# xipengwang/AprilSAM

Hardware: AMD Instinct MI355X
Metric: Gauss-Newton iterations/sec + factorise ms on M3500 (chi2 match <=1e-6) (higher is better)
Workload: dtype f64; 1 GPU; M3500 batch april_graph_cholesky, 1 replica per GPU (3500 poses, 5454 factors, n=10500); parallelism=single GPU, fronts=680, levels=9, nnz_L=422121

## Files before the change

### aprilsam_amd/csrc/capi.cpp

```cpp
#include <cstdio>
#include <cstdlib>
#include <cstring>
#include <string>
#include <vector>

#include "../../include/aprilsam_amd.h"
#include "plan.h"
#include "errors.h"
#include "refmodel.h"
#include "solver.h"

extern "C" {

void APRILSAM_VERSION(void) {
    printf("================\n");
    printf("| APRILSAM 0.0 |   solver: aprilsam_amd (MI355X / gfx950)\n");
    printf("================\n");
    printf("\n");
}

void april_graph_cholesky_param_init(april_graph_cholesky_param_t *param) {
    asam::drop_context(param);
    asam::unbind_param(param);
    memset(param, 0, sizeof(*param));
    param->tikhanov = 0.0001;
    param->nreordering = 1;
    asam::warm_up();
}

void april_graph_cholesky_param_destory(april_graph_cholesky_param_t *param) {
    if (!param) return;
    asam::drop_context(param);
    asam::unbind_param(param);
    free(param->delta_x); free(param->B); free(param->y); free(param->ordering);
    free(param);
}

void april_graph_cholesky(april_graph_t *graph, april_graph_cholesky_param_t *param) { asam::batch_step(graph, param); }

void april_graph_cholesky_inc(april_graph_t *graph, april_graph_cholesky_param_t *param) { asam::inc_step(graph, param); }

void april_graph_cholesky_inc_solver(april_graph_t *graph, april_graph_cholesky_param_t *param, int *idxs) {
    (void)idxs;
    asam::inc_solve_only(graph, param);
}

double april_graph_chi2(april_graph_t *graph) { return asam::graph_chi2(graph); }

int aprilsam_amd_device_count(void) { return asam::api_device_count(); }
int aprilsam_amd_set_device(int device) { return asam::api_set_device(device); }
int aprilsam_amd_param_set_device(const april_graph_cholesky_param_t *param, int slot) { return asam::api_param_set_device(param, slot); }
int aprilsam_amd_param_get_device(const april_graph_cholesky_param_t *param) { return asam::api_param_get_device(param); }
int aprilsam_amd_set_option(const char *name, double value) { return asam::api_set_option(name, value); }
int aprilsam_amd_debug_guard_selftest(const april_graph_cholesky_param_t *param) { return asam::debug_guard_selftest(param); }
int aprilsam_amd_get_option(const char *name, double *value) { return asam::api_get_option(name, value); }
int aprilsam_amd_get_stats(const april_graph_cholesky_param_t *param, aprilsam_amd_stats_t *out) {
    return asam::get_stats(param, out) ? 0 : -1;
}
int aprilsam_amd_batch_resident(april_graph_t *graph, april_graph_cholesky_param_t *param, int iters, double *chi2_out, double *ms_out) {
    return asam::batch_resident(graph, param, iters, chi2_out, ms_out);
}
int aprilsam_amd_resident_begin(april_graph_t *graph, april_graph_cholesky_param_t *param) { return asam::resident_begin(graph, param); }
int aprilsam_amd_resident_steps(april_graph_t *graph, april_graph_cholesky_param_t *param, int n, int mode) { return asam::resident_steps(graph, param, n, mode); }
int aprilsam_amd_resident_sync(april_graph_t *graph, april_graph_cholesky_param_t *param) { return asam::resident_sync(graph, param); }
double aprilsam_amd_resident_chi2(april_graph_t *graph) { return asam::resident_chi2(graph); }
int aprilsam_amd_resident_end(april_graph_t *graph, april_graph_cholesky_param_t *param) { return asam::resident_end(graph, param); }
int aprilsam_amd_level_profile(const april_graph_cholesky_param_t *param, double *out6, int cap_levels) { return asam::level_profile(param, out6, cap_levels); }
int aprilsam_amd_kernel_profile(const april_graph_cholesky_param_t *param, double *ms, long long *calls, double *flops, double *bytes, const char **names) {
    return asam::kernel_profile(param, ms, calls, flops, bytes, names);
}
int aprilsam_amd_debug_stage(april_graph_t *graph, april_graph_cholesky_param_t *param, int what, double *out) { return asam::debug_stage(graph, param, what, out); }
int aprilsam_amd_debug_front_times(const april_graph_cholesky_param_t *param, long long *out, int n_fronts) { return asam::debug_front_times(param, out, n_fronts); }
int aprilsam_amd_reference_order(int n_nodes, int n_factors, const int *fa, const int *fb, int *out_order, int *out_parent) {
    asam::RefModel m;
    m.batch(n_nodes, n_factors, fa, fb);
    memcpy(out_order, m.ord.data(), sizeof(int) * (size_t)n_nodes);
    if (out_parent) memcpy(out_parent, m.parent.data(), sizeof(int) * (size_t)n_nodes);
    return 0;
}
int aprilsam_amd_shard_begin(april_graph_t *graph, april_graph_cholesky_param_t *param, int rank, int world) { return asam::shard_begin(graph, param, rank, world); }
long long aprilsam_amd_shard_info(const april_graph_cholesky_param_t *param, int what, long long *out, long long cap) { return asam::shard_info(param, what, out, cap); }
int aprilsam_amd_shard_comm_unique_id(char *out128) { return asam::shard_comm_unique_id(out128); }
int aprilsam_amd_shard_comm_init_rccl(april_graph_cholesky_param_t *param, const char *id128) { return asam::shard_comm_init_rccl(param, id128); }
int aprilsam_amd_shard_comm_init_host(april_graph_cholesky_param_t *param, const aprilsam_amd_host_comm_t *cb) { return asam::shard_comm_init_host(param, cb); }
int aprilsam_amd_shard_comm_info(const april_graph_cholesky_param_t *param, long long *out5, char *rccl_path, int cap) { return asam::shard_comm_info(param, out5, rccl_path, cap); }
int aprilsam_amd_shard_iterate(april_graph_t *graph, april_graph_cholesky_param_t *param, int n) { return asam::shard_iterate(graph, param, n); }
int aprilsam_amd_shard_gather_states(april_graph_t *graph, april_graph_cholesky_param_t *param) { return asam::shard_gather_states(graph, param); }
double aprilsam_amd_shard_chi2(april_graph_t *graph, april_graph_cholesky_param_t *param) { return asam::shard_chi2(graph, param); }
void aprilsam_amd_shard_end(april_graph_cholesky_param_t *param) { asam::shard_end(param); }

void *aprilsam_amd_refmodel_create(void) { return new asam::RefModel(); }
void aprilsam_amd_refmodel_destroy(void *m) { delete (asam::RefModel *)m; }
void aprilsam_amd_refmodel_batch(void *m, int n_nodes, int n_factors, const int *fa, const int *fb) { ((asam::RefModel *)m)->batch(n_nodes, n_factors, fa, fb); }
int aprilsam_amd_refmodel_inc_begin(void *m, int n_nodes, int n_factors, const int *fa, const int *fb) {
    asam::RefModel *M = (asam::RefModel *)m;
    M->inc_begin(n_nodes, n_factors, fa, fb);
    return M->naffected;
}
int aprilsam_amd_refmodel_solve_visit(void *m, const double *x, double dxy, double dth, int *visited) {
    asam::RefModel *M = (asam::RefModel *)m;
    for (int i = 0; i < M->N; i++) visited[i] = 0;
    M->solve_visit(x, dxy, dth, [&](int n, bool upd) { visited[n] = upd ? 2 : 1; });
    return M->start_over;
}
void aprilsam_amd_refmodel_get(void *m, int *parent, int *changed, int *relin) {
    asam::RefModel *M = (asam::RefModel *)m;
    for (int i = 0; i < M->N; i++) { if (parent) parent[i] = M->parent[i]; if (changed) changed[i] = M->changed[i]; if (relin) relin[i] = M->relin[i]; }
}
int aprilsam_amd_refmodel_check(void *m) { return ((asam::RefModel *)m)->check_tree(); }
int aprilsam_amd_last_error(char *msg, int cap) { return asam::get_last_error(msg, cap); }
void aprilsam_amd_clear_error(void) { asam::clear_last_error(); }
int aprilsam_amd_selftest(void) { return asam::selftest(); }
const char *aprilsam_amd_version(void) { return "aprilsam_amd 0.1 (gfx950, multifrontal FP64)"; }
void aprilsam_amd_free(void *p) { free(p); }

struct aprilsam_amd_plan { asam::Plan P; };

aprilsam_amd_plan_t *aprilsam_amd_plan_create(int n_nodes, int n_factors, const int *factor_nodes, const double *xy, int leaf_nodes) {
    aprilsam_amd_plan *pl = new aprilsam_amd_plan();
    try {
        asam::build_plan(pl->P, n_nodes, n_factors, factor_nodes, xy, leaf_nodes > 0 ? leaf_nodes : asam::g_opt.leaf_nodes);
    } catch (const asam::SolverError &e) {
        asam::set_last_error(e.code, e.msg);
        fprintf(stderr, "aprilsam_amd: ERROR %d: %s\n", e.code, e.msg.c_str());
        delete pl;
        return nullptr;
    } catch (const std::exception &e) {
        asam::set_last_error(asam::ERR_INTERNAL, e.what());
        fprintf(stderr, "aprilsam_amd: ERROR %d: %s\n", (int)asam::ERR_INTERNAL, e.what());
        delete pl;
        return nullptr;
    }
    return pl;
}
void aprilsam_amd_plan_destroy(aprilsam_amd_plan_t *plan) { delete plan; }

long long aprilsam_amd_shard_plan(const aprilsam_amd_plan_t *plan, int world, int what, long long *out, long long cap) {
    if (!plan || world < 1) return -1;
    std::vector<int> owner; std::vector<char> top; std::vector<long long> xfer, bcast, v;
    asam::shard_map(plan->P, world, owner, top, xfer, bcast);
    if (what == 1) v = xfer; else if (what == 2) v = bcast; else if (what == 3) v.assign(owner.begin(), owner.end());
    else if (what == 4) v = asam::shard_critical_path(plan->P, world, owner, top); else return -1;
    if (out) for (long long i = 0; i < (long long)v.size() && i < cap; i++) out[i] = v[i];
    return (long long)v.size();
}

long long aprilsam_amd_plan_query(const aprilsam_amd_plan_t *plan, const char *what, long long **out) {
    std::string k(what);
    if (k.compare(0, 3, "bd_") == 0 || k.compare(0, 3, "rd_") == 0) asam::build_gather_lists(const_cast<asam::Plan &>(plan->P));
    const asam::Plan &P = plan->P;
    std::vector<long long> v;
    auto from = [&](const auto &a) { v.assign(a.begin(), a.end()); };
    if (k == "perm") from(P.perm);
    else if (k == "pos") from(P.pos);
    else if (k == "front_first") from(P.f_first);
    else if (k == "front_nsb") from(P.f_nsb);
    else if (k == "front_nub") from(P.f_nub);
    else if (k == "front_parent") from(P.f_parent);
    else if (k == "front_level") from(P.f_level);
    else if (k == "front_rows_ptr") from(P.f_rows_ptr);
    else if (k == "front_rows") from(P.f_rows);
    else if (k == "front_rel") from(P.f_rel);
    else if (k == "front_off") from(P.f_off);
    else if (k == "ch_ptr") from(P.ch_ptr);
    else if (k == "ch_idx") from(P.ch_idx);
    else if (k == "factor_front") from(P.fac_front);
    else if (k == "factor_la") from(P.fac_la);
    else if (k == "factor_lb") from(P.fac_lb);
    else if (k == "factor_swap") from(P.fac_swap);
    else if (k == "bd_front_ptr") from(P.bd_front_ptr);
    else if (k == "bd_row") from(P.bd_row);
    else if (k == "bd_col") from(P.bd_col);
    else if (k == "bd_src_ptr") from(P.bd_src_ptr);
    else if (k == "bd_src") from(P.bd_src);
    else if (k == "rd_front_ptr") from(P.rd_front_ptr);
    else if (k == "rd_col") from(P.rd_col);
    else if (k == "rd_src_ptr") from(P.rd_src_ptr);
    else if (k == "rd_src") from(P.rd_src);
    else if (k == "lev_ptr") from(P.lev_ptr);
    else if (k == "lev_fronts") from(P.lev_fronts);
    else if (k == "stats") v = { P.nF, P.nLevels, P.max_rows, (long long)P.nnzL, (long long)P.flops, (long long)P.pool_doubles };
    else { *out = nullptr; return -1; }
    *out = (long long *)malloc(sizeof(long long) * (v.size() + 1));
    if (!v.empty()) memcpy(*out, v.data(), sizeof(long long) * v.size());
    return (long long)v.size();
}

}
```

### aprilsam_amd/csrc/kernels.hip.h

```cpp
#pragma once
#include <hip/hip_runtime.h>
#include <stdint.h>

#include <type_traits>
namespace asam {

constexpr int PROF_SLOTS = 16;
constexpr int TPB = 256;
constexpr int NB = 32;
constexpr int TILE = 64;
constexpr int ASM_CB = 4;
constexpr int OBP = 4;

struct FrontDesc {
    long long off;
    int nsb, nub, first;
    int dest_begin, dest_end;
    int ch_begin, ch_end;
    int rows_begin;
    int parent;
    int dinv0;
    int prim1, prim2;
    int pad[2];
};
static_assert(sizeof(FrontDesc) == 64, "FrontDesc must stay one cache line");
struct DestRec { int brow, bcol, src_begin, src_end; };
struct ChildRec {
    long long uoff;
    int cR;
    int cnu;
    int rel_begin;
    int pad;
};
static_assert(sizeof(ChildRec) == 24, "ChildRec layout");

struct DevPlan {
    int nF;
    const FrontDesc *fd;
    const DestRec *dest;
    const ChildRec *child;
    const int *f_rows, *f_rel;
    const int *slot_blk, *slot_rhs;
    const int *src_idx;
    const double *lambda;
    long long *prof;
    int prof_mode;
    int schur_first_nub;
    int *epoch; const int *flevel; int l0; const int *marks;
};

__host__ __device__ inline int asm_chunks(int nbc) { return (nbc + ASM_CB - 1) / ASM_CB; }
struct SyrkRange { int k_lo, k_hi, col_lo, col_hi, ntr, ntc; };
__host__ __device__ inline SyrkRange syrk_range(int R, int C, int ns, int s_lo, int s_hi, int tile = TILE, bool ahead = false) {
    SyrkRange g;
    g.k_lo = s_lo * NB;
    g.k_hi = s_hi * NB < ns ? s_hi * NB : ns;
    g.col_lo = g.k_hi;
    g.col_hi = ahead ? (g.k_hi + OBP * NB < ns ? g.k_hi + OBP * NB : ns) : C;
    if (g.k_hi <= g.k_lo || g.col_hi <= g.col_lo) { g.ntr = g.ntc = 0; return g; }
    g.ntr = ((R - 2) - g.col_lo + tile - 1) / tile;
    g.ntc = (g.col_hi - g.col_lo + tile - 1) / tile;
    return g;
}
__host__ __device__ inline int syrk_tiles(int R, int C, int ns, int s_lo, int s_hi, int tile = TILE, bool ahead = false) {
    SyrkRange g = syrk_range(R, C, ns, s_lo, s_hi, tile, ahead);
    return g.ntc * g.ntr - g.ntc * (g.ntc - 1) / 2;
}
__device__ __forceinline__ int find_seg(const int *__restrict__ pre, int n, int bid) {
    int lo = 0, hi = n;
    while (hi - lo > 1) { int m = (lo + hi) >> 1; if (pre[m] <= bid) lo = m; else hi = m; }
    return lo;
}

__device__ __forceinline__ void trapezoid_tile(int l, int ntr, int ntc, int *ti, int *tj_);
constexpr int SYRK_SB = 8;
constexpr int SYRK_MODE_XCD_SHIFT = 8;
__host__ __device__ inline void trapezoid_tile_xcd(int l, int nt, int ntr, int ntc, int *ti, int *tj) {
    const int q = nt >> 3, rem = nt & 7, x = l & 7;
    int lp = x * q + (x < rem ? x : rem) + (l >> 3);
    for (int c0 = 0;; ) {
        const int w = ntc - c0 < SYRK_SB ? ntc - c0 : SYRK_SB;
        const int cnt = w * (ntr - c0) - w * (w - 1) / 2;
        if (lp < cnt || c0 + w >= ntc) {
            const int tri = w * (w + 1) / 2;
            if (lp < tri) { int r = 0; while ((r + 1) * (r + 2) / 2 <= lp) r++; *ti = c0 + r; *tj = c0 + lp - r * (r + 1) / 2; }
            else { const int e = lp - tri; *ti = c0 + w + e / w; *tj = c0 + e % w; }
            return;
        }
        lp -= cnt; c0 += w;
    }
// ... 735 lines not shown
        }
    }
}
template <int BWT>
__device__ __forceinline__ void chain_store_diag(double *S, int ld, int k0, int wdt, const double (&Dd)[BWT]) {
    const int r = threadIdx.x & 63;
    if (r < wdt) {
#pragma unroll
        for (int c = 0; c < BWT; c++) if (c < wdt) S[(k0 + c) * ld + k0 + r] = (c <= r) ? Dd[c] : 0.0;
    }
}
template <int NT>
__device__ __forceinline__ void factor_dense_blk(double *S, int ld, int ns, int Rv, int hi, int *bad, double * , long long *pf = nullptr) {
    constexpr int NW = NT / 64;
    long long t_chain = 0, t_syrk = 0, t0 = 0;
    const int wave = __builtin_amdgcn_readfirstlane(threadIdx.x >> 6);
    auto chain_sync_store = [&](int k0, int nwc) {
        const int wdt = min(BW, ns - k0);
        if (wdt <= 8) {
            double D8[8];
            chain_block<NT, 8>(S, ld, k0, wdt, Rv, bad, D8, nwc);
            __syncthreads();
            if (wave == 0) chain_store_diag<8>(S, ld, k0, wdt, D8);
        } else {
            double D16[16];
            chain_block<NT, 16>(S, ld, k0, wdt, Rv, bad, D16, nwc);
            __syncthreads();
            if (wave == 0) chain_store_diag<16>(S, ld, k0, wdt, D16);
        }
    };
    auto chain_waves = [&](int k0) {
        const int wdt = min(BW, ns - k0), brows = 64 - (wdt <= 8 ? 8 : 16);
        const int nchunk = max(1, (Rv - (k0 + wdt) + brows - 1) / brows);
        return min(nchunk, NW / 2);
    };
    if (pf) t0 = wall_clock64();
    chain_sync_store(0, NW);
    if (pf) { const long long t1 = wall_clock64(); t_chain += t1 - t0; t0 = t1; }
    for (int k0 = 0; k0 < ns; k0 += BW) {
        const int wdt = min(BW, ns - k0), below0 = k0 + wdt;
        if (below0 < ns) {
            const int next_hi = min(below0 + BW, ns), cw = chain_waves(below0);
            if (NW >= 8) lds_syrk16<NT>(S, ld, k0, below0, below0, next_hi, Rv, 1, NW - 1);
            else lds_syrk16<NT>(S, ld, k0, below0, below0, next_hi, Rv);
            __syncthreads();
            if (pf) { const long long t1 = wall_clock64(); t_syrk += t1 - t0; t0 = t1; }
            if (wave < cw) {
                long long w0_ = 0, c0_ = 0;
                if (pf) { w0_ = wall_clock64(); c0_ = clock64(); }
                chain_sync_store(below0, cw);
                if (pf && threadIdx.x == 0) { pf[10] += clock64() - c0_; pf[15] += wall_clock64() - w0_; }
            } else {
                if (next_hi < hi) lds_syrk16<NT>(S, ld, k0, below0, next_hi, hi, Rv, cw, NW - cw);
                __syncthreads();
            }
            if (pf) { const long long t1 = wall_clock64(); t_chain += t1 - t0; t0 = t1; }
        } else {
            __syncthreads();
            if (below0 < hi) lds_syrk16<NT>(S, ld, k0, below0, below0, hi, Rv);
            __syncthreads();
            if (pf) { const long long t1 = wall_clock64(); t_syrk += t1 - t0; t0 = t1; }
        }
    }
    if (pf && threadIdx.x == 0) { pf[8] = t_chain; pf[9] = t_syrk; }
}
template <int NT>
__device__ __forceinline__ void factor_front_blk(double *S, int ld, int nsb, int nbc, int *bad, double *stage, int nbc_upd = -1, long long *pf = nullptr) {
    if (nbc_upd < 0) nbc_upd = nbc;
    factor_dense_blk<NT>(S, ld, 3 * nsb, 3 * (nbc + 1) - 2, 3 * nbc_upd, bad, stage, pf);
}

__host__ __device__ inline size_t small_front_lds(int R, int C, int nw) { return (size_t)(R | 1) * C * 8 + wl_bytes(nw); }
__host__ __device__ inline size_t panel_front_lds(int R, int ns, int nw) { return (size_t)(R | 1) * ns * 8 + wl_bytes(nw); }

template <int NT>
__device__ __forceinline__ void front_small_body(const DevPlan &P, const int t, double *__restrict__ pool, const double *__restrict__ Hc, int *bad,
                                                 long long full_lds_limit, int *flags, int wait, double *S) {
    const int *wflags = wait ? flags : nullptr;
    const int ev = flags ? flag_value(P) : 0;
    const FrontDesc D = P.fd[t];
    const int nsb = D.nsb, nbc = D.nsb + D.nub;
    const int R = 3 * (nbc + 1), C = 3 * nbc, ld = R | 1;
    double *Fg = pool + D.off;
    if ((long long)small_front_lds(R, C, NT / 64) <= full_lds_limit) {
        int2 *wl = (int2 *)(S + (size_t)ld * C);
        if (P.prof && threadIdx.x == 0) P.prof[(size_t)t * PROF_SLOTS + 0] = wall_clock64();
        assemble_front<NT, ASM_LDS>(P, D, pool, Hc, 0, nbc, true, S, ld, nullptr, 0, wl, P.prof ? P.prof + (size_t)t * PROF_SLOTS : nullptr, wflags, bad, ev);
        if (P.prof && threadIdx.x == 0) P.prof[(size_t)t * PROF_SLOTS + 1] = wall_clock64();
        factor_front_blk<NT>(S, ld, nsb, nbc, bad, (double *)wl, -1, P.prof ? P.prof + (size_t)t * PROF_SLOTS : nullptr);
        if (P.prof && threadIdx.x == 0) P.prof[(size_t)t * PROF_SLOTS + 2] = wall_clock64();
        for (int c = 3 * nsb + (threadIdx.x >> 6); c < C; c += NT / 64) {
            int r0 = 3 * (c / 3);
            for (int r = r0 + (threadIdx.x & 63); r < R; r += 64) Fg[(size_t)c * R + r] = S[(size_t)c * ld + r];
        }
        if (flags) publish_flag(flags + t, ev);
        for (int c = threadIdx.x >> 6; c < 3 * nsb; c += NT / 64) {
            int r0 = 3 * (c / 3);
            for (int r = r0 + (threadIdx.x & 63); r < R; r += 64) Fg[(size_t)c * R + r] = S[(size_t)c * ld + r];
        }
    } else {
        const int ns = 3 * nsb;
        int2 *wl = (int2 *)(S + (size_t)ld * ns);
        const bool schur_first = P.schur_first_nub > 0 && D.nub >= P.schur_first_nub;
        if (P.prof && threadIdx.x == 0) P.prof[(size_t)t * PROF_SLOTS + 0] = wall_clock64();
        if (schur_first) assemble_front<NT, ASM_SPLIT>(P, D, pool, Hc, 0, nsb, false, S, ld, Fg, R, wl, P.prof ? P.prof + (size_t)t * PROF_SLOTS : nullptr, wflags, bad, ev);
        else assemble_front<NT, ASM_SPLIT>(P, D, pool, Hc, 0, nbc, true, S, ld, Fg, R, wl, P.prof ? P.prof + (size_t)t * PROF_SLOTS : nullptr, wflags, bad, ev);
        if (P.prof && threadIdx.x == 0) P.prof[(size_t)t * PROF_SLOTS + 1] = wall_clock64();
        factor_front_blk<NT>(S, ld, nsb, nbc, bad, (double *)wl, nsb, P.prof ? P.prof + (size_t)t * PROF_SLOTS : nullptr);
        if (P.prof && threadIdx.x == 0) P.prof[(size_t)t * PROF_SLOTS + 2] = wall_clock64();
        if (schur_first) {
            lds_panel_syrk<NT, 2>(S, ld, 0, ns, ns, C, R - 2, Fg, R);
            __syncthreads();
            assemble_front<NT, ASM_GLOBAL, false>(P, D, pool, Hc, nsb, nbc, false, nullptr, 0, Fg, R, wl, nullptr, nullptr, bad);
        }
        else if (nbc > nsb) lds_panel_syrk<NT, 1>(S, ld, 0, ns, ns, C, R - 2, Fg, R);
        if (flags) publish_flag(flags + t, ev);
        for (int c = threadIdx.x >> 6; c < ns; c += NT / 64) {
            int r0 = 3 * (c / 3);
            for (int r = r0 + (threadIdx.x & 63); r < R; r += 64) Fg[(size_t)c * R + r] = S[(size_t)c * ld + r];
        }
    }
    if (P.prof) { __syncthreads(); if (threadIdx.x == 0) P.prof[(size_t)t * PROF_SLOTS + 3] = wall_clock64(); }
}
constexpr int UPD_MAXF = 4;
constexpr int UPD_MAXC = 4;
struct UpdRec {
    long long old_off;
    int mode;
    int old_nub;
    int wout;
    int mask;
    int n_own, own_f[UPD_MAXF], own_la[UPD_MAXF], own_lb[UPD_MAXF], own_slot[UPD_MAXF];
    int n_ch, ch_t[UPD_MAXC], ch_wout[UPD_MAXC], ch_rel[UPD_MAXC], ch_cnu[UPD_MAXC], ch_mask[UPD_MAXC];
    int pad[3];
};
static_assert(sizeof(UpdRec) == 192, "UpdRec layout");
struct UpdCtx {
    const UpdRec *recs;
    double *wbuf;
    int *wflags;
    const int *fa, *fb; const double *Z, *Wm, *lp, *st;
};
__host__ __device__ inline size_t update_front_lds(int R, int ns, int nact) {
    return (size_t)((size_t)ns * (R | 1) + (size_t)3 * nact * (R | 1) + 8 * ns + 3 * (ns | 1) + 16) * 8;
}
template <int NT>
__device__ __forceinline__ void front_update_body(const DevPlan &P, const int t, const UpdRec &rec, const UpdCtx &uc, double *__restrict__ pool,
                                                  int *flags, int *bad, double *S) {
    constexpr int NW = NT / 64;
    const FrontDesc D = P.fd[t];
    const int tid = threadIdx.x, wave = __builtin_amdgcn_readfirstlane(tid >> 6), lane = tid & 63;
    const int ns = 3 * D.nsb, nu = 3 * D.nub, m = ns + nu, R = m + 3, ld = R | 1;
    const int nu_o = 3 * rec.old_nub, m_o = ns + nu_o, R_o = m_o + 3;
    const double *Fo = pool + rec.old_off;
    double *Fg = pool + D.off;
    const int nact = __popc(rec.mask), wld = nu + 1, nsp = ns | 1;
    double *Ls = S;
    double *Wv = Ls + (size_t)ns * ld;
    double *K8 = Wv + (size_t)3 * nact * ld;
    double *Wa = K8 + 8 * ns;
    double *Cm = Wa + 3 * nsp;
    long long *pf = P.prof ? P.prof + (size_t)t * PROF_SLOTS : nullptr;
    if (pf && tid == 0) pf[0] = wall_clock64();
    const int ev = (flags || uc.wflags) ? flag_value(P) : 0;
    {
        const int ne = ns * R;
// ... 170 lines not shown
#pragma unroll
                    for (int u = 0; u < 4; u++) { L[u] = Li[(size_t)(j + u) * ld]; pp[3 * u] = K8[8 * (j + u)]; pp[3 * u + 1] = K8[8 * (j + u) + 1]; pp[3 * u + 2] = K8[8 * (j + u) + 2]; }
#pragma unroll
                    for (int u = 0; u < 4; u++) { r0 = fma(-L[u], pp[3 * u], r0); r1 = fma(-L[u], pp[3 * u + 1], r1); r2 = fma(-L[u], pp[3 * u + 2], r2); }
                }
                for (; j < ns; j++) { const double L = Li[(size_t)j * ld]; r0 = fma(-L, K8[8 * j], r0); r1 = fma(-L, K8[8 * j + 1], r1); r2 = fma(-L, K8[8 * j + 2], r2); }
                const double w0 = r0 * Cm[0], w1 = (r1 - Cm[1] * w0) * Cm[2], w2 = (r2 - Cm[3] * w0 - Cm[4] * w1) * Cm[5];
                wo[i - ns] = w0; wo[(size_t)wld + i - ns] = w1; wo[(size_t)2 * wld + i - ns] = w2;
            }
        }
        if (si == nact - 1 && uc.wflags) {
            if (pf && tid == 0) pf[2] = wall_clock64();
            publish_flag(uc.wflags + t, ev);
        } else __syncthreads();
        {
            for (int i = tid; i <= m; i += NT) {
                double r0 = W0[i], r1 = W0[(size_t)ld + i], r2 = W0[(size_t)2 * ld + i];
                const int jn = min(i + 1, ns);
                double *Li = Ls + i;
                int j = 0;
                for (; j + 4 <= jn; j += 4) {
                    double L[4], kk[28];
#pragma unroll
                    for (int u = 0; u < 4; u++) {
                        L[u] = Li[(size_t)(j + u) * ld];
#pragma unroll
                        for (int v = 0; v < 7; v++) kk[7 * u + v] = K8[8 * (j + u) + v];
                    }
#pragma unroll
                    for (int u = 0; u < 4; u++) {
                        r0 = fma(-L[u], kk[7 * u], r0); r1 = fma(-L[u], kk[7 * u + 1], r1); r2 = fma(-L[u], kk[7 * u + 2], r2);
                        L[u] = fma(kk[7 * u + 6], L[u], fma(r0, kk[7 * u + 3], fma(r1, kk[7 * u + 4], r2 * kk[7 * u + 5])));
                    }
#pragma unroll
                    for (int u = 0; u < 4; u++) Li[(size_t)(j + u) * ld] = L[u];
                }
                for (; j < jn; j++) {
                    const double *k8 = K8 + 8 * j;
                    const double L = Li[(size_t)j * ld];
                    r0 = fma(-L, k8[0], r0); r1 = fma(-L, k8[1], r1); r2 = fma(-L, k8[2], r2);
                    Li[(size_t)j * ld] = fma(k8[6], L, fma(r0, k8[3], fma(r1, k8[4], r2 * k8[5])));
                }
                if (i >= ns) {
                    const double w0 = r0 * Cm[0], w1 = (r1 - Cm[1] * w0) * Cm[2], w2 = (r2 - Cm[3] * w0 - Cm[4] * w1) * Cm[5];
                    W0[i] = w0; W0[(size_t)ld + i] = w1; W0[(size_t)2 * ld + i] = w2;
                }
            }
        }
        __syncthreads();
    }
    for (int cu0 = 4 * wave; cu0 < nu; cu0 += 4 * NW) {
        for (int pass = 0; pass * 64 < nu + 1; pass++) {
            double old[4];
#pragma unroll
            for (int u = 0; u < 4; u++) {
                const int cu = min(cu0 + u, nu - 1), ru = pass * 64 + lane;
                const bool has = cu < nu_o && (ru < nu_o || ru == nu);
                old[u] = has ? Fo[(size_t)(ns + cu) * R_o + ns + (ru == nu ? nu_o : ru)] : 0.0;
            }
#pragma unroll
            for (int u = 0; u < 4; u++) {
                const int cu = cu0 + u, ru = pass * 64 + lane;
                if (cu < nu && ru <= nu && ru >= 3 * (cu / 3)) {
                    double acc = old[u];
                    for (int v = 0; v < 3 * nact; v++) acc = fma(Wv[(size_t)v * ld + ns + ru], Wv[(size_t)v * ld + ns + cu], acc);
                    Fg[(size_t)(ns + cu) * R + ns + ru] = acc;
                }
            }
        }
    }
    for (int c = wave; c < ns; c += NW) {
        const int r0 = 3 * (c / 3);
        for (int r = r0 + lane; r < R; r += 64) Fg[(size_t)c * R + r] = Ls[(size_t)c * ld + r];
    }
    if (flags) publish_flag(flags + t, ev);
    if (pf) { __syncthreads(); if (tid == 0) pf[3] = wall_clock64(); }
}

template <int NT>
__global__ void __launch_bounds__(NT) k_front_small(DevPlan P, const int *__restrict__ fronts, double *__restrict__ pool,
                                                    const double *__restrict__ Hc, int *bad, long long full_lds_limit,
                                                    int *flags = nullptr, int wait = 0, UpdCtx uc = UpdCtx{}) {
    extern __shared__ __attribute__((aligned(16))) double S[];
    if (uc.recs) {
        const UpdRec *rec = uc.recs + blockIdx.x;
        if (rec->mode) { front_update_body<NT>(P, fronts[blockIdx.x], *rec, uc, pool, flags, bad, S); return; }
    }
    front_small_body<NT>(P, fronts[blockIdx.x], pool, Hc, bad, full_lds_limit, flags, wait, S);
}

constexpr int ASM_INV_CAP = 4096;
__global__ void __launch_bounds__(TPB) k_assemble_big(DevPlan P, const int *__restrict__ list, const int *__restrict__ pre, int n,
                                                      double *__restrict__ pool, const double *__restrict__ Hc) {
    const int a = find_seg(pre, n, blockIdx.x);
    const int t = list[a], bc0 = (blockIdx.x - pre[a]) * ASM_CB;
    const FrontDesc D = P.fd[t];
    const int nbc = D.nsb + D.nub;
    const int bc1 = min(bc0 + ASM_CB, nbc);
    __shared__ int2 wl[wl_bytes(TPB / 64) / 8];
    __shared__ short inv[2][ASM_INV_CAP];
    const int prim = D.prim1 - 1, sec = D.prim2 - 1;
    if (prim < 0 || nbc + 1 > ASM_INV_CAP) {
        assemble_front<TPB, ASM_GLOBAL>(P, D, pool, Hc, bc0, bc1, false, nullptr, 0, pool + D.off, 3 * (nbc + 1), wl);
        return;
    }
    const int tid = threadIdx.x, wv = __builtin_amdgcn_readfirstlane(tid >> 6), lane = tid & 63;
    const int nst = sec >= 0 ? 2 : 1;
    const ChildRec cr0 = P.child[D.ch_begin + prim], cr1 = P.child[D.ch_begin + max(sec, 0)];
    const int R = 3 * (nbc + 1);
    for (int e = tid; e <= nbc; e += TPB) { inv[0][e] = -1; inv[1][e] = -1; }
    __syncthreads();
    for (int j = tid; j < cr0.cnu; j += TPB) inv[0][P.f_rel[cr0.rel_begin + j]] = (short)j;
    if (nst > 1) for (int j = tid; j < cr1.cnu; j += TPB) inv[1][P.f_rel[cr1.rel_begin + j]] = (short)j;
    if (tid == 0) { inv[0][nbc] = (short)cr0.cnu; if (nst > 1) inv[1][nbc] = (short)cr1.cnu; }
    __syncthreads();
    double *__restrict__ dst = pool + D.off;
    for (int col = 3 * bc0 + wv; col < 3 * bc1; col += TPB / 64) {
        const int bcol = col / 3, c3 = col - 3 * bcol;
        const double lam = col < 3 * D.nsb ? P.lambda[D.first + bcol] : 0.0;
        const int jc0 = __builtin_amdgcn_readfirstlane((int)inv[0][bcol]), jc1 = nst > 1 ? __builtin_amdgcn_readfirstlane((int)inv[1][bcol]) : -1;
        if (jc0 < 0 && jc1 < 0) {
            for (int row = 3 * bcol + lane; row < R; row += 64) dst[(size_t)col * R + row] = row == col ? lam : 0.0;
            continue;
        }
        const int cc0 = 3 * max(jc0, 0) + c3, cc1 = 3 * max(jc1, 0) + c3;
        const double *__restrict__ s0 = pool + cr0.uoff + (size_t)cc0 * cr0.cR, *__restrict__ s1 = pool + cr1.uoff + (size_t)cc1 * cr1.cR;
        for (int r0 = 3 * bcol; r0 < R; r0 += 128) {
            double v0[2], v1[2]; bool ok0[2], ok1[2];
#pragma unroll
            for (int u = 0; u < 2; u++) {
                const int row = r0 + 64 * u + lane, rc = min(row, R - 1), brow = rc / 3, i3 = rc - 3 * brow;
                const int jr0 = inv[0][brow], cr_0 = 3 * jr0 + i3, jr1 = inv[1][brow], cr_1 = 3 * jr1 + i3;
                ok0[u] = row < R && jc0 >= 0 && jr0 >= 0 && (brow < nbc ? cr_0 >= cc0 : i3 == 0);
                ok1[u] = row < R && jc1 >= 0 && jr1 >= 0 && (brow < nbc ? cr_1 >= cc1 : i3 == 0);
                v0[u] = ld_agent(s0 + (ok0[u] ? cr_0 : cc0));
                v1[u] = ld_agent(s1 + (ok1[u] ? cr_1 : cc1));
            }
#pragma unroll
            for (int u = 0; u < 2; u++) {
                const int row = r0 + 64 * u + lane;
                if (row < R) dst[(size_t)col * R + row] = ((row == col ? lam : 0.0) + (ok0[u] ? v0[u] : 0.0)) + (ok1[u] ? v1[u] : 0.0);
            }
        }
    }
    __syncthreads();
    assemble_front<TPB, ASM_GLOBAL, false>(P, D, pool, Hc, bc0, bc1, false, nullptr, 0, dst, R, wl, nullptr, nullptr, nullptr, 0, prim, sec);
}

__device__ __forceinline__ void rsq_stage(int st, double dn, double &y, double &h, double &e) {
    if (st == 0) { y = __builtin_amdgcn_rsq(dn); h = 0.5 * dn; }
    else if (st == 1 || st == 4) e = -h * y;
    else if (st == 2 || st == 5) e = fma(e, y, 0.5);
    else if (st == 3 || st == 6) y = fma(y, e, y);
}
__device__ __forceinline__ void diag_chain32(double (&D)[NB], int r, int &isbad, double &myinv) {
    double dn = readlane_d(D[0], 0);
    if (!(dn > 0)) isbad = 1;
    double inv = fast_rsqrt(dn);
#pragma unroll
    for (int j = 0; j < NB; j++) {
        D[j] *= inv;
        myinv = (r == j) ? inv : myinv;
        double y = 0, h = 0, e = 0;
        if (j + 1 < NB) {
            const double l1 = readlane_d(D[j], j + 1);
            D[j + 1] = fma(-D[j], l1, D[j + 1]);
            dn = readlane_d(D[j + 1], j + 1);
            isbad = (dn > 0) ? isbad : 1;
        }
#pragma unroll
        for (int gi = 0; gi < 2; gi++) {
// ... 393 lines not shown
    const int seg = find_seg(pre, n, blockIdx.x);
    const int t = list[seg], cb = blockIdx.x - pre[seg];
    const FrontDesc D_ = P.fd[t];
    const int nsb = D_.nsb, nub = D_.nub, nbc = nsb + nub;
    const int R = 3 * (nbc + 1), ns = 3 * nsb, nu = 3 * nub;
    const int k0 = cb * NB, wdt = min(NB, ns - k0);
    const double *Fg = pool + D_.off;
    const int tid = threadIdx.x, wave = tid >> 6, lane = tid & 63;
    const int *rows = P.f_rows + D_.rows_begin;
    const int c0 = wave * 8;
    double acc[8];
    const double *colp[8];
#pragma unroll
    for (int q = 0; q < 8; q++) { acc[q] = 0; colp[q] = Fg + (size_t)(k0 + min(c0 + q, wdt - 1)) * R + ns; }
    for (int r0 = 0; r0 < nu; r0 += BS_CHUNK) {
        const int nr = min(BS_CHUNK, nu - r0);
        __syncthreads();
        for (int e = tid; e < nr; e += TPB) xu[e] = x[(size_t)3 * rows[(r0 + e) / 3] + (r0 + e) % 3];
        __syncthreads();
        int i = lane;
        for (; i + 192 < nr; i += 256) {
            double v[4][8];
#pragma unroll
            for (int u = 0; u < 4; u++)
#pragma unroll
                for (int q = 0; q < 8; q++) v[u][q] = colp[q][r0 + i + 64 * u];
#pragma unroll
            for (int u = 0; u < 4; u++) {
                const double xv = xu[i + 64 * u];
#pragma unroll
                for (int q = 0; q < 8; q++) acc[q] = fma(v[u][q], xv, acc[q]);
            }
        }
        for (; i < nr; i += 64) {
            const double xv = xu[i];
#pragma unroll
            for (int q = 0; q < 8; q++) acc[q] = fma(colp[q][r0 + i], xv, acc[q]);
        }
    }
#pragma unroll
    for (int q = 0; q < 8; q++) {
        const double sum = wave_sum63(acc[q]);
        if (lane == 63 && c0 + q < wdt) x[(size_t)3 * D_.first + k0 + c0 + q] = sum;
    }
}

__host__ __device__ inline size_t backsolve_lds(int m, int ns, bool pre) { return (size_t)(m + NB + 8 + NB * (NB + 1) + (pre ? (size_t)ns * ((m + 3) | 1) : 0)) * 8; }
struct UpdArgs { const int *perm; const double *lp; double *st, *dX, *st_out, *dx_out; int *bad_out; double *lp_next; };
__device__ __forceinline__ void backsolve_finish(const FrontDesc &D_, int t, const double *xw, double *__restrict__ x, int *xflags, int *bad, const UpdArgs &upd, int ev = 0) {
    const int tid = threadIdx.x, nsb = D_.nsb, ns = 3 * nsb;
    for (int e = tid; e < ns; e += TPB) x[(size_t)3 * D_.first + e] = xw[e];
    if (xflags) publish_flag(xflags + t, ev);
    if (upd.perm) {
        for (int k = tid; k < nsb; k += TPB) {
            const int i = upd.perm[D_.first + k];
            const double d0 = xw[3 * k], d1 = xw[3 * k + 1], d2 = xw[3 * k + 2];
            if (isnan(d0) || isnan(d1) || isnan(d2)) {
                const double qnan = __longlong_as_double(0x7ff8000000000000ll);
                upd.dX[3 * i + 0] = qnan; upd.dX[3 * i + 1] = qnan; upd.dX[3 * i + 2] = qnan;
                if (upd.dx_out) { upd.dx_out[3 * i + 0] = qnan; upd.dx_out[3 * i + 1] = qnan; upd.dx_out[3 * i + 2] = qnan; }
                continue;
            }
            const double s0 = upd.lp[3 * i + 0] + d0, s1 = upd.lp[3 * i + 1] + d1, s2 = mod2pi_dev(upd.lp[3 * i + 2] + d2);
            if (upd.st) { upd.st[3 * i + 0] = s0; upd.st[3 * i + 1] = s1; upd.st[3 * i + 2] = s2; }
            if (upd.lp_next) { upd.lp_next[3 * i + 0] = s0; upd.lp_next[3 * i + 1] = s1; upd.lp_next[3 * i + 2] = s2; }
            upd.dX[3 * i + 0] = d0; upd.dX[3 * i + 1] = d1; upd.dX[3 * i + 2] = d2;
            if (upd.st_out) {
                upd.st_out[3 * i + 0] = s0; upd.st_out[3 * i + 1] = s1; upd.st_out[3 * i + 2] = s2;
                upd.dx_out[3 * i + 0] = d0; upd.dx_out[3 * i + 1] = d1; upd.dx_out[3 * i + 2] = d2;
            }
        }
    }
    if (upd.bad_out && tid == 0 && __hip_atomic_load(bad, __ATOMIC_RELAXED, __HIP_MEMORY_SCOPE_AGENT) != 0) {
#pragma unroll
        for (int k = 0; k < 4; k++) upd.bad_out[k] = __hip_atomic_load(bad + k, __ATOMIC_RELAXED, __HIP_MEMORY_SCOPE_AGENT);
    }
}
constexpr int BS_TALL_ROWS = 768;
template <bool PRE, bool TALL = false>
__global__ void __launch_bounds__(TPB) k_backsolve_t(DevPlan P, const int *__restrict__ fronts, const double *__restrict__ pool,
                                                     double *__restrict__ x, int split, int *xflags, int wait, int *bad, UpdArgs upd) {
    extern __shared__ __attribute__((aligned(16))) double smem[];
    const int t = fronts[blockIdx.x];
    const int ev = xflags ? flag_value(P) : 0;
    const FrontDesc D_ = P.fd[t];
    const int nsb = D_.nsb, nub = D_.nub, nbc = nsb + nub;
    const int R = 3 * (nbc + 1), ns = 3 * nsb, m = 3 * nbc;
    double *xw = smem;
    double *part = smem + m;
    double *Ldg = smem + m + NB + 8;
    const double *Fg = pool + D_.off;
    const int tid = threadIdx.x, wave = tid >> 6, lane = tid & 63;
    const int *rows = P.f_rows + D_.rows_begin;
    long long *pf = (P.prof && P.prof_mode == 2) ? P.prof + (size_t)t * PROF_SLOTS : nullptr;
    double *Lp = smem + m + NB + 8 + NB * (NB + 1);
    const int ldp = R | 1;
    auto Lat = [&](int c, int r) -> double { if constexpr (PRE) return Lp[c * ldp + r]; else return Fg[(size_t)c * R + r]; };
    if constexpr (PRE) {
        const int ne = ns * R;
        for (int e0 = tid; e0 < ne; e0 += 8 * TPB) {
            double v[8];
#pragma unroll
            for (int u = 0; u < 8; u++) v[u] = Fg[min(e0 + u * TPB, ne - 1)];
#pragma unroll
            for (int u = 0; u < 8; u++) { const int e = e0 + u * TPB; if (e < ne) { const int c = e / R; Lp[c * ldp + (e - c * R)] = v[u]; } }
        }
    }
    if (wait && D_.parent >= 0) {
        if (tid == 0) wait_flag(xflags + D_.parent, bad, ev);
        if constexpr (PRE) { __syncthreads(); asm volatile("" ::: "memory"); }
        else acquire_all();
    }
    if (pf && tid == 0) pf[4] = wall_clock64();
    const bool pre_t = split && bs_split_front(nsb, nub);
    const int mprod = pre_t ? ns : m;
    if (pre_t) { for (int e = tid; e < ns; e += TPB) xw[e] = Fg[(size_t)e * R + m] - x[(size_t)3 * D_.first + e]; }
    else {
        for (int e = tid; e < ns; e += TPB) xw[e] = Fg[(size_t)e * R + m];
        for (int e = tid; e < 3 * nub; e += TPB) { const double *xp = x + (size_t)3 * rows[e / 3] + e % 3; if constexpr (PRE) xw[ns + e] = ld_agent(xp); else xw[ns + e] = *xp; }
    }
    __syncthreads();
    if (pf && tid == 0) pf[5] = wall_clock64();
    long long t_prod = 0, t_sum = 0, t_solve = 0, ts = 0;
    constexpr int PFU = 8;
    double pv[TALL ? PFU : 1][8], pdg[4];
    auto prefetch = [&](int k1p) {
        if constexpr (TALL && !PRE) {
            const int k0p = max(0, k1p - NB), wdtp = k1p - k0p;
#pragma unroll
            for (int q = 0; q < 4; q++) {
                const int e = tid + q * TPB, r = e & 31, cc = e >> 5;
                pdg[q] = Fg[(size_t)(k0p + min(cc, wdtp - 1)) * R + k0p + min(r, wdtp - 1)];
            }
#pragma unroll
            for (int u = 0; u < PFU; u++) {
                const int row = min(k1p + lane + 64 * u, mprod - 1);
                if (k1p + 64 * u < mprod) {
#pragma unroll
                    for (int q = 0; q < 8; q++) pv[u][q] = Fg[(size_t)(k0p + min(wave * 8 + q, wdtp - 1)) * R + row];
                } else {
#pragma unroll
                    for (int q = 0; q < 8; q++) pv[u][q] = 0.0;
                }
            }
        }
    };
    prefetch(ns);
    for (int k1 = ns; k1 > 0; k1 -= NB) {
        const int k0 = max(0, k1 - NB), wdt = k1 - k0;
        if (pf) ts = wall_clock64();
        double dg[4];
#pragma unroll
        for (int q = 0; q < 4; q++) {
            const int e = tid + q * TPB, r = e & 31, cc = e >> 5;
            if constexpr (TALL && !PRE) dg[q] = pdg[q]; else dg[q] = Lat(k0 + min(cc, wdt - 1), k0 + min(r, wdt - 1));
        }
        {
            const int c0 = wave * 8;
            double acc[8];
            int colc[8];
#pragma unroll
            for (int q = 0; q < 8; q++) { acc[q] = 0; colc[q] = k0 + min(c0 + q, wdt - 1); }
            int i = k1 + lane;
            if constexpr (TALL && !PRE) {
                {
                    double xv[PFU];
// ... 158 lines not shown
        Gemv128 g;
        const int wnext = B < nB - 1 ? min(OBW, ns - (k0 + OBW)) : 1;
        if (B < nB - 1) gemv128_load(g, Fg, R, k0 + OBW, wnext, k0);
        if (B < nB - 2 && tid == 0) wait_flag(tflag + B, bad);
#pragma unroll
        for (int k = 0; k < 24; k++) {
            const int e = tid + TPB * k, bq = e >> 10, i = e & 31, j = (e >> 5) & 31;
            const int sr = bq == 0 ? 1 : (bq < 3 ? 2 : 3);
            Ls[bq * (NB * (NB + 1)) + i * (NB + 1) + j] = (NB * sr + i < Wb) ? lv[k] : 0.0;
        }
#pragma unroll
        for (int k = 0; k < 16; k++) { const int e = tid + TPB * k; Iv[(e >> 10) * (NB * (NB + 1)) + ((e >> 5) & 31) * (NB + 1) + (e & 31)] = iv[k]; }
        if (B < nB - 1) gemv128_sums(g, w, [&](int q, double sum) { xs[32 * wave + q] = sum; });
        __syncthreads();
        {
            double v = 0.0;
            const int e = tid;
            if (e < Wb) {
                v = Fg[(size_t)(k0 + e) * R + m] - xw[k0 + e];
                if (B < nB - 1) v -= xs[e];
                if (B < nB - 2) v -= ld_agent(farf + (size_t)B * OBW + e);
            }
            __syncthreads();
            if (e < OBW) w[e] = v;
        }
        __syncthreads();
        for (int sb = nsub - 1; sb >= 0; sb--) {
            {
                const int i = tid & 31, part = tid >> 5;
                double acc = 0;
#pragma unroll
                for (int jj = 0; jj < 4; jj++) { const int j = 4 * part + jj; acc = fma(Iv[sb * (NB * (NB + 1)) + j * (NB + 1) + i], w[NB * sb + j], acc); }
                xs[part * NB + i] = acc;
            }
            __syncthreads();
            if (tid < NB) {
                double v = 0;
#pragma unroll
                for (int part = 0; part < 8; part++) v += xs[part * NB + tid];
                w[NB * sb + tid] = v;
                if (NB * sb + tid < Wb) xw[k0 + NB * sb + tid] = v;
            }
            __syncthreads();
            if (sb > 0) {
                const int q = tid >> 6, l = tid & 63, j = l & 31, half = l >> 5;
                if (q < sb) {
                    const int bq = (sb == 1 ? 0 : (sb == 2 ? 1 : 3)) + q;
                    double acc = 0;
#pragma unroll
                    for (int ii = 0; ii < 16; ii++) { const int i = 16 * half + ii; acc = fma(Ls[bq * (NB * (NB + 1)) + i * (NB + 1) + j], w[NB * sb + i], acc); }
                    xs[256 + (q * 2 + half) * NB + j] = acc;
                }
                __syncthreads();
                if (tid < NB * sb) { const int q = tid >> 5, j = tid & 31; w[NB * q + j] -= xs[256 + (q * 2) * NB + j] + xs[256 + (q * 2 + 1) * NB + j]; }
                __syncthreads();
            }
        }
        for (int e = tid; e < Wb; e += TPB) x[(size_t)3 * D_.first + k0 + e] = xw[k0 + e];
        if (B >= 2 && H > 0) publish_flag(xflag + B);
    }
    __syncthreads();
    for (int e = tid; e < 2 * BSB_MAXB; e += TPB) reset_flag(xflag + e, 0);
    backsolve_finish(D_, t, xw, x, nullptr, bad, upd);
}

constexpr int BSW = 64;
constexpr int BSW_MAX_NS = NB + 8 + NB * (NB + 1) - 256;
template <int BSWT = BSW>
__device__ __forceinline__ void backsolve_w_body(const DevPlan &P, const int t, const double *__restrict__ pool, double *__restrict__ x, int *xflags, int *bad,
                                                 const UpdArgs &upd, double *smem) {
    const int ev = xflags ? flag_value(P) : 0;
    const FrontDesc D_ = P.fd[t];
    const int nsb = D_.nsb, nub = D_.nub, nbc = nsb + nub;
    const int R = 3 * (nbc + 1), ns = 3 * nsb, m = 3 * nbc;
    double *xw = smem;
    double *partial = smem + m;
    double *dgs = smem + m + 256;
    double *Lp = smem + m + NB + 8 + NB * (NB + 1);
    const int ldp = R | 1;
    const double *Fg = pool + D_.off;
    const int tid = threadIdx.x, wave = tid >> 6, lane = tid & 63;
    const int *rows = P.f_rows + D_.rows_begin;
    long long *pf = (P.prof && P.prof_mode == 2) ? P.prof + (size_t)t * PROF_SLOTS : nullptr;
    {
        const int ne = ns * R;
        for (int e0 = tid; e0 < ne; e0 += 8 * TPB) {
            double v[8];
#pragma unroll
            for (int u = 0; u < 8; u++) v[u] = Fg[min(e0 + u * TPB, ne - 1)];
#pragma unroll
            for (int u = 0; u < 8; u++) {
                const int e = e0 + u * TPB;
                if (e < ne) {
                    const int c = e / R, r = e - c * R;
                    Lp[c * ldp + r] = r > c ? v[u] : 0.0;
                    if (r == c) dgs[c] = v[u];
                }
            }
        }
    }
    if (xflags && D_.parent >= 0) {
        if (tid == 0) wait_flag(xflags + D_.parent, bad, ev);
        __syncthreads();
        asm volatile("" ::: "memory");
       
    }
    if (pf && tid == 0) pf[4] = wall_clock64();
    for (int e = tid; e < ns; e += TPB) xw[e] = Fg[(size_t)e * R + m];
    for (int e = tid; e < 3 * nub; e += TPB) xw[ns + e] = ld_agent(x + (size_t)3 * rows[e / 3] + e % 3);
    __syncthreads();
    if (pf && tid == 0) pf[5] = wall_clock64();
    for (int k1 = ns; k1 > 0; k1 -= BSWT) {
        const int k0 = max(0, k1 - BSWT), wdt = k1 - k0;
        const bool on = lane < wdt;
        const int c = k0 + (on ? lane : 0);
        const double *Lc = Lp + (size_t)c * ldp;
        auto chain = [&](auto w_) {
            constexpr int W = decltype(w_)::value;
            double l[W];
#pragma unroll
            for (int i = 1; i < W; i++) l[i] = Lc[k0 + min(i, wdt - 1)];
            const double rinv = on ? 1.0 / dgs[c] : 1.0;
#pragma unroll
            for (int i = 1; i < W; i++) l[i] *= rinv;
            __syncthreads();
            if (pf && tid == 0 && k1 == ns) pf[6] = wall_clock64();
            double w = on ? (xw[c] - ((partial[64 + lane] + partial[128 + lane]) + partial[192 + lane])) * rinv : 0.0;
#pragma unroll
            for (int i = W - 1; i > 0; i--) {
                const double xi = readlane_d(w, i);
                w = fma(-l[i], xi, w);
            }
            if (on) xw[c] = w;
        };
        if (wave == 0) {
            if (wdt <= 16) chain(std::integral_constant<int, 16>{});
            else if (BSWT <= 32 || wdt <= 32) chain(std::integral_constant<int, 32>{});
            else if constexpr (BSWT > 32) chain(std::integral_constant<int, 64>{});
        } else {
            double acc0 = 0, acc1 = 0;
            int i = k1 + wave - 1;
            for (; i + 3 < m; i += 6) { acc0 = fma(Lc[i], xw[i], acc0); acc1 = fma(Lc[i + 3], xw[i + 3], acc1); }
            if (i < m) acc0 = fma(Lc[i], xw[i], acc0);
            partial[wave * 64 + lane] = acc0 + acc1;
            __syncthreads();
        }
        __syncthreads();
    }
    if (pf && tid == 0) pf[7] = wall_clock64();
    backsolve_finish(D_, t, xw, x, xflags, bad, upd, ev);
}
__global__ void __launch_bounds__(TPB) k_backsolve_w(DevPlan P, const int *__restrict__ fronts, const double *__restrict__ pool,
                                                     double *__restrict__ x, int *xflags, int *bad, UpdArgs upd) {
    extern __shared__ __attribute__((aligned(16))) double smem[];
    backsolve_w_body(P, fronts[blockIdx.x], pool, x, xflags, bad, upd, smem);
}

__host__ __device__ inline long long upd_packed_offset(int R, int ns, int j) {
    const long long Rv = R - 2, nb0 = ns / 3, b = j / 3, e = j - 3 * b;
    return 3 * ((b - nb0) * Rv - 3 * (nb0 + b - 1) * (b - nb0) / 2) + e * (Rv - 3 * b);
}
__global__ void __launch_bounds__(TPB) k_guard(int mode, const long long *__restrict__ offs, int n, int len, double *__restrict__ pool, int *count) {
    const int b = blockIdx.x;
    if (b >= n) return;
    unsigned long long *g = (unsigned long long *)(pool + offs[b]);
    int bad = 0;
    for (int i = threadIdx.x; i < len; i += TPB) {
        if (mode == 0) g[i] = ~0ull;
        else if (g[i] != ~0ull) bad++;
    }
    if (bad) { atomicAdd(count, bad); count[1] = b; }
}
__global__ void __launch_bounds__(TPB) k_poison(DevPlan P, const int *__restrict__ list, int n, const int *__restrict__ skip_mode, int skip_stride, int what,
                                                double *__restrict__ pool, double *__restrict__ x) {
    if ((int)blockIdx.x >= n) return;
    if (skip_mode && skip_mode[(size_t)blockIdx.x * skip_stride]) return;
    const int t = list ? list[blockIdx.x] : (int)blockIdx.x;
    const FrontDesc D = P.fd[t];
    const int nbc = D.nsb + D.nub, R = 3 * (nbc + 1), ns = 3 * D.nsb, C = 3 * nbc;
    const double qnan = __longlong_as_double(0x7ff8000000000000ll);
    double *Fg = pool + D.off;
    if (what & 1)
        for (int c = ns + (threadIdx.x >> 6); c < C; c += TPB / 64)
            for (int r = 3 * (c / 3) + (threadIdx.x & 63); r < R - 2; r += 64) Fg[(size_t)c * R + r] = qnan;
    if (what & 2) for (int e = threadIdx.x; e < ns; e += TPB) x[(size_t)3 * D.first + e] = qnan;
}
__global__ void __launch_bounds__(TPB) k_pack_update(double *__restrict__ front, int R, int ns, double *__restrict__ buf, int dir) {
    const int j = ns + blockIdx.x, Rv = R - 2, r0 = j / 3 * 3;
    double *__restrict__ col = front + (size_t)j * R;
    double *__restrict__ pk = buf + upd_packed_offset(R, ns, j) - r0;
    if (dir == 0) { for (int r = r0 + threadIdx.x; r < Rv; r += TPB) pk[r] = col[r]; }
    else { for (int r = r0 + threadIdx.x; r < Rv; r += TPB) col[r] = pk[r]; }
}

struct Patch { void *dst; long long src_off; long long bytes; };
__global__ void __launch_bounds__(TPB) k_apply_patches(const Patch *__restrict__ patches, const char *__restrict__ payload) {
    const Patch p = patches[blockIdx.x];
    const char *src = payload + p.src_off;
    char *dst = (char *)p.dst;
    if (((((size_t)dst) | ((size_t)src) | (size_t)p.bytes) & 3) == 0) {
        for (long long i = threadIdx.x; i < p.bytes / 4; i += TPB) ((int *)dst)[i] = ((const int *)src)[i];
    } else {
        for (long long i = threadIdx.x; i < p.bytes; i += TPB) dst[i] = src[i];
    }
}
struct IncFlags { int *epoch; int *marks; const int *up_list; int n_up; };
constexpr int INL_PATCHES = 24, INL_BYTES = 2048;
struct alignas(16) InlinePatches { Patch hdr[INL_PATCHES]; char pay[INL_BYTES]; };
struct IncPrologue {
    const Patch *patches; const char *payload; int n_patch, f_begin, f_end;
    int inl;

    const int *fa, *fb; const double *Z, *Wm, *lp, *st; const unsigned char *swp; const int *slot_blk, *slot_rhs; double *Hc; int *bad;
    long long *stamps;
    int *done; int seq;
};
struct IncArgsHead { IncPrologue a; IncFlags fl; InlinePatches inl; };
constexpr int TAIL_MAXF = 8;
__device__ __forceinline__ void inc_prologue_body(const IncPrologue &a, const IncFlags &fl, double *mirror = nullptr) {
    const Patch *patches = a.patches; const char *payload = a.payload; const int n_patch = a.n_patch, f_begin = a.f_begin, f_end = a.f_end;
    const int *__restrict__ fa = a.fa, *__restrict__ fb = a.fb; const double *__restrict__ Z = a.Z, *__restrict__ Wm = a.Wm, *__restrict__ lp = a.lp, *__restrict__ st = a.st;
    const unsigned char *__restrict__ swp = a.swp; const int *__restrict__ slot_blk = a.slot_blk, *__restrict__ slot_rhs = a.slot_rhs; double *__restrict__ Hc = a.Hc; int *__restrict__ bad = a.bad;
    const int wave = threadIdx.x >> 6, lane = threadIdx.x & 63, nthr = (int)blockDim.x;
    if (threadIdx.x < 4) bad[threadIdx.x] = 0;
    const char *kargs = (const char *)__builtin_amdgcn_kernarg_segment_ptr() + offsetof(IncArgsHead, inl);
    if (a.inl) { patches = (const Patch *)(kargs + offsetof(InlinePatches, hdr)); payload = kargs + offsetof(InlinePatches, pay); }
    for (int q = wave; q < n_patch; q += nthr >> 6) {
        const Patch p = patches[q];
        const char *src = payload + p.src_off;
        char *dst = (char *)p.dst;
        if (((((size_t)dst) | ((size_t)src) | (size_t)p.bytes) & 3) == 0) {
            const int nw = (int)(p.bytes / 4);
            for (int i0 = lane; i0 < nw; i0 += 512) {
                int v[8];
#pragma unroll
                for (int u = 0; u < 8; u++) v[u] = ((const int *)src)[min(i0 + 64 * u, nw - 1)];
#pragma unroll
                for (int u = 0; u < 8; u++) if (i0 + 64 * u < nw) ((int *)dst)[i0 + 64 * u] = v[u];
// ... 243 lines not shown
```

### aprilsam_amd/csrc/plan.h

```cpp
#pragma once
#include <cstdint>
#include <functional>
#include <vector>

namespace asam {

struct Plan {
    int N = 0;
    int F = 0;
    int leaf_nodes = 16;

    std::vector<int> perm;
    std::vector<int> pos;

    int nF = 0;
    std::vector<int> f_first;
    std::vector<int> f_nsb;
    std::vector<int> f_nub;
    std::vector<int> f_parent;
    std::vector<int> f_level;
    std::vector<int64_t> f_rows_ptr;
    std::vector<int> f_rows;
    std::vector<int> f_rel;
    std::vector<int> ch_ptr, ch_idx;
    std::vector<int64_t> f_off;
    int64_t pool_doubles = 0;

    inline int rows(int t) const { return 3 * (f_nsb[t] + f_nub[t] + 1); }
    inline int cols(int t) const { return 3 * (f_nsb[t] + f_nub[t]); }

    std::vector<int> fac_front;
    std::vector<int> fac_la, fac_lb;
    std::vector<int> bd_front_ptr;
    std::vector<int> bd_row, bd_col;
    std::vector<int> bd_src_ptr;
    std::vector<int> bd_src;
    std::vector<int> rd_front_ptr;
    std::vector<int> rd_col;
    std::vector<int> rd_src_ptr;
    std::vector<int> rd_src;
    std::vector<uint8_t> fac_swap;
    struct DestRec { int brow, bcol, src_begin, src_end; };
    std::vector<int> dest_front_ptr;
    std::vector<DestRec> dest;
    std::vector<int> slot_blk;
    std::vector<int> slot_rhs;
    int n_slots = 0;

    int nLevels = 0;
    std::vector<int> lev_ptr, lev_fronts;

    int max_rows = 0;
    int64_t nnzL = 0;
    double flops = 0;
};

void build_plan(Plan &P, int N, int F, const int *factor_nodes, const double *xy, int leaf_nodes);
void build_gather_lists(Plan &P);

struct NDTree {
    struct Node { std::vector<int> verts; std::vector<int> children; };
    std::vector<Node> nodes;
    std::vector<int> roots;
};
void nested_dissection(int N, const std::vector<int> &adj_ptr, const std::vector<int> &adj,
                       const double *xy, int leaf_nodes, NDTree &tree);

struct PlanSession { explicit PlanSession(int n_nodes, int min_nodes = 1024); ~PlanSession(); PlanSession(const PlanSession &) = delete; bool on = false; };
void plan_parallel_for(int n, int grain, const std::function<void(int, int)> &body);

}
```

### aprilsam_amd/csrc/solver.h

```cpp
#pragma once
#include <vector>
#include "../../include/aprilsam_amd.h"

namespace asam {

struct Options {
    int leaf_nodes = 16;
    int deterministic = 0;
    int use_graph = 1;
    int device_timing = 0;
    int trust_factor_cache = 0;
    int small_lds_kb = 156;
    int inc_fast = 1;
    int inc_multi = 1;
    int inc_one = 1;
    int inc_one_up = 3, inc_one_dn = 4, inc_one_threads = 512, inc_one_spin = 1;
    int inc_tail = 1;
    int inc_inline = 1;
    int inc_tail_solve = 1;
    int inc_lazy_states = 1;
    int inc_replan_tall = 1;
    int inc_update = 1;
    int speculate_factors = 1;
    int warm_up = 1;
    int syrk_xcd_order = 512;
    int syrk_small_tiles = 320;
    int syrk_pair_tiles = 2048;
    int syrk_group = 3;
    int schur_first = 40;
    int small_threads = 1024;
    int tp_threads = 512;
    int tp_fronts = 1000;
    int tp_lds_kb = 80;
    int amalg = 0;
    int amalg_max = 64;
    int pin_last = 0;
    int batch_extend = 1;
    int extend_tail_fronts = 3;
    int persist = 1;
    int persist_max_fronts = 240;
    int tail_poses = 28;
    int blk_backsolve = 1;
    int wave_backsolve = 1;
    int linearize_staged_min = 32768;
    int mem_cap_mb = 0;
    int pool_guard = 0;
    int pool_poison = 0;
    int skip_flag_waits = 0;
    int panel_mode = 1;
};
extern Options g_opt;

void batch_step(april_graph_t *g, april_graph_cholesky_param_t *param);
void inc_step(april_graph_t *g, april_graph_cholesky_param_t *param);
void inc_solve_only(april_graph_t *g, april_graph_cholesky_param_t *param);
double graph_chi2(april_graph_t *g);
int batch_resident(april_graph_t *g, april_graph_cholesky_param_t *param, int iters, double *chi2_out, double *ms_out);
int resident_begin(april_graph_t *g, april_graph_cholesky_param_t *param);
int resident_steps(april_graph_t *g, april_graph_cholesky_param_t *param, int n, int mode);
int resident_sync(april_graph_t *g, april_graph_cholesky_param_t *param);
double resident_chi2(april_graph_t *g);
int resident_end(april_graph_t *g, april_graph_cholesky_param_t *param);
int level_profile(const april_graph_cholesky_param_t *param, double *out, int cap_levels);
int kernel_profile(const april_graph_cholesky_param_t *param, double *ms, long long *calls, double *flops, double *bytes, const char **names);
void drop_context(const april_graph_cholesky_param_t *p);
void drop_graph_pack(const april_graph_t *g);
bool get_stats(const april_graph_cholesky_param_t *p, aprilsam_amd_stats_t *out);
int shard_begin(april_graph_t *g, april_graph_cholesky_param_t *param, int rank, int world);
long long shard_info(const april_graph_cholesky_param_t *param, int what, long long *out, long long cap);
int shard_comm_unique_id(char *out128);
int shard_comm_init_rccl(const april_graph_cholesky_param_t *param, const char *id128);
int shard_comm_init_host(const april_graph_cholesky_param_t *param, const aprilsam_amd_host_comm_t *cb);
int shard_comm_info(const april_graph_cholesky_param_t *param, long long *out, char *path, int cap);
int shard_iterate(april_graph_t *g, april_graph_cholesky_param_t *param, int n);
int shard_gather_states(april_graph_t *g, april_graph_cholesky_param_t *param);
double shard_chi2(april_graph_t *g, april_graph_cholesky_param_t *param);
void shard_end(const april_graph_cholesky_param_t *param);
int debug_guard_selftest(const april_graph_cholesky_param_t *param);
int debug_stage(april_graph_t *g, april_graph_cholesky_param_t *param, int what, double *out);
int debug_front_times(const april_graph_cholesky_param_t *param, long long *out, int n_fronts);
int api_device_count();
int selftest();
struct Plan;
void shard_map(const Plan &P, int world, std::vector<int> &owner, std::vector<char> &top, std::vector<long long> &xfer, std::vector<long long> &bcast);
std::vector<long long> shard_critical_path(const Plan &P, int world, const std::vector<int> &owner, const std::vector<char> &top);
int api_set_device(int d);
int api_param_set_device(const april_graph_cholesky_param_t *param, int slot);
int api_param_get_device(const april_graph_cholesky_param_t *param);
void unbind_param(const april_graph_cholesky_param_t *param);
void warm_up() noexcept;
int api_set_option(const char *name, double v);
int api_get_option(const char *name, double *v);
int marginals(april_graph_t *g, april_graph_cholesky_param_t *param, int n, const int *qa, const int *qb, double *cov, bool joint);
long long selinv_runs(const april_graph_cholesky_param_t *param);
int marginals_joint_any(april_graph_t *g, april_graph_cholesky_param_t *param, int n, const int *a, const int *b, double *cov);
int gate_xyt(april_graph_t *g, april_graph_cholesky_param_t *param, int n, const int *a, const int *b, const double *z, const double *W, double *d2, double *S);
long long path_solve_bytes(const april_graph_cholesky_param_t *param);
int max_selected(april_graph_t *g, april_graph_cholesky_param_t *param, int n, const int *factors, int *out);
void lm_opts_init(aprilsam_amd_lm_opts_t *opts);
int optimize_lm(april_graph_t *g, april_graph_cholesky_param_t *param, const aprilsam_amd_lm_opts_t *opts, aprilsam_amd_lm_report_t *report, double *trace);
constexpr int MAX_MIX_K = 8;
bool is_native_max(const april_graph_factor_t *f);
bool max_check(const april_graph_factor_t *f, char *why, int cap);
double max_const(const april_graph_factor_t *f, int i);
int max_select(const april_graph_factor_t *f, const double *pa, const double *pb);
bool robust_of(const april_graph_factor_t *f, int *kind, double *c);
double robust_host_s(const double *z, const double *w, const double *pa, const double *pb);
int robust_weights(april_graph_t *g, april_graph_cholesky_param_t *param, int n, const int *factors, double *w);

}
```

### aprilsam_amd/csrc/solver.hip.cpp

```cpp
#include <hip/hip_runtime.h>
#include <rccl/rccl.h>
#include <dlfcn.h>

#include <algorithm>
#include <array>
#include <chrono>
#include <thread>
#include <cmath>
#include <cstdio>
#include <cstdlib>
#include <cstring>
#include <map>
#include <memory>
#include <atomic>
#include <mutex>
#include <string>
#include <unordered_map>
#include <vector>

#include "../../include/aprilsam_amd.h"
#include "errors.h"
#include "kernels.hip.h"
#include "maxmix.hip.h"
#include "robust.hip.h"
#include "lm.hip.h"
#include "selinv.hip.h"
#include "pathsolve.hip.h"
#include "plan.h"
#include "refmodel.h"
#include "solver.h"

namespace asam {

#define HIPCHECK(expr)                                                                                 \
    do {                                                                                               \
        hipError_t e_ = (expr);                                                                        \
        if (e_ != hipSuccess) {                                                                        \
            (void)hipGetLastError();                                                                   \
            fail(e_ == hipErrorOutOfMemory ? ERR_OOM : ERR_HIP, "%s failed: %s (%s:%d)", #expr, hipGetErrorString(e_), __FILE__, __LINE__); \
        }                                                                                              \
    } while (0)

static double now_ms() {
    return std::chrono::duration<double, std::milli>(std::chrono::steady_clock::now().time_since_epoch()).count();
}

Options g_opt;
struct OptionDef { const char *name; int Options::*member; int min_value; bool policy; int max_value = 0x7fffffff; };
static const OptionDef OPTION_TABLE[] = {
    { "leaf_nodes", &Options::leaf_nodes, 1, false }, { "deterministic", &Options::deterministic, 0, true }, { "use_graph", &Options::use_graph, 0, true },
    { "device_timing", &Options::device_timing, 0, true }, { "trust_factor_cache", &Options::trust_factor_cache, 0, true },
    { "small_lds_kb", &Options::small_lds_kb, 0, false }, { "syrk_xcd_order", &Options::syrk_xcd_order, 0, false },
    { "schur_first", &Options::schur_first, 0, false }, { "syrk_small_tiles", &Options::syrk_small_tiles, 0, false }, { "syrk_pair_tiles", &Options::syrk_pair_tiles, 0, false }, { "syrk_group", &Options::syrk_group, 2, false, 8 }, { "panel_mode", &Options::panel_mode, 0, false },
    { "small_threads", &Options::small_threads, 64, false }, { "tp_fronts", &Options::tp_fronts, 0, false }, { "tp_lds_kb", &Options::tp_lds_kb, 0, false },
    { "tp_threads", &Options::tp_threads, 64, false }, { "inc_fast", &Options::inc_fast, 0, true }, { "inc_multi", &Options::inc_multi, 0, true },
    { "inc_one", &Options::inc_one, 0, true }, { "inc_one_up", &Options::inc_one_up, 1, true }, { "inc_one_dn", &Options::inc_one_dn, 1, true },
    { "inc_one_threads", &Options::inc_one_threads, 64, true }, { "inc_one_spin", &Options::inc_one_spin, 0, true }, { "inc_tail", &Options::inc_tail, 0, false },
    { "inc_inline", &Options::inc_inline, 0, true }, { "inc_update", &Options::inc_update, 0, true }, { "inc_tail_solve", &Options::inc_tail_solve, 0, true },
    { "inc_lazy_states", &Options::inc_lazy_states, 0, true }, { "inc_replan_tall", &Options::inc_replan_tall, 0, true },
    { "speculate_factors", &Options::speculate_factors, 0, true }, { "warm_up", &Options::warm_up, 0, true }, { "pin_last", &Options::pin_last, 0, false }, { "persist", &Options::persist, 0, false },
    { "persist_max_fronts", &Options::persist_max_fronts, 0, false }, { "linearize_staged_min", &Options::linearize_staged_min, 0, false },
    { "wave_backsolve", &Options::wave_backsolve, 0, false }, { "blk_backsolve", &Options::blk_backsolve, 0, false }, { "tail_poses", &Options::tail_poses, 8, false },
    { "batch_extend", &Options::batch_extend, 0, true }, { "extend_tail_fronts", &Options::extend_tail_fronts, 0, true }, { "mem_cap_mb", &Options::mem_cap_mb, 0, true },
    { "pool_guard", &Options::pool_guard, 0, false }, { "amalg", &Options::amalg, 0, false }, { "amalg_max", &Options::amalg_max, 1, false }, { "pool_poison", &Options::pool_poison, 0, false }, { "skip_flag_waits", &Options::skip_flag_waits, 0, false },
};
static const OptionDef *find_option(const char *name) {
    for (const OptionDef &d : OPTION_TABLE) if (!strcmp(d.name, name)) return &d;
    return nullptr;
}
static std::once_flag g_opt_once;
static void load_env_options() {
    std::call_once(g_opt_once, [] {
        for (const OptionDef &d : OPTION_TABLE) {
            std::string env = "APRILSAM_AMD_";
            for (const char *q = d.name; *q; q++) env += (char)toupper((unsigned char)*q);
            const char *sv = getenv(env.c_str());
            if (sv && *sv) g_opt.*(d.member) = std::min(d.max_value, std::max(d.min_value, (int)atof(sv)));
        }
    });
}

constexpr int MAX_SLOTS = 64;
static std::atomic<int> g_device{ -1 };
static std::mutex g_slot_mu[MAX_SLOTS];
static thread_local int t_slot = 0;
static int device_count() {
    static std::atomic<int> cached{ 0 };
    int n = cached.load(std::memory_order_relaxed);
    if (n > 0) return n;
    if (hipGetDeviceCount(&n) != hipSuccess) { (void)hipGetLastError(); return 0; }
    if (n > 0) cached.store(n, std::memory_order_relaxed);
    return n;
}
static int physical_device(int slot) { const int n = device_count(); return n > 0 ? slot % n : 0; }
static thread_local int t_device = -1;
template <class V> struct Registry {
    using Map = std::map<const void *, std::unique_ptr<V>>;
    Map m; mutable std::mutex mu;
    typename Map::iterator find(const void *k) { std::lock_guard<std::mutex> lk(mu); return m.find(k); }
    typename Map::iterator end() { return m.end(); }
    std::pair<typename Map::iterator, bool> emplace(const void *k, std::unique_ptr<V> v) { std::lock_guard<std::mutex> lk(mu); return m.emplace(k, std::move(v)); }
    void erase(typename Map::iterator it) { std::lock_guard<std::mutex> lk(mu); m.erase(it); }
    void put(const void *k, std::unique_ptr<V> v) { std::lock_guard<std::mutex> lk(mu); m[k] = std::move(v); }
    template <class F> void for_each(F &&f) { std::lock_guard<std::mutex> lk(mu); for (auto &kv : m) f(*kv.second); }
    template <class F> bool with(const void *k, F &&f) { std::lock_guard<std::mutex> lk(mu); auto it = m.find(k); if (it == m.end()) return false; f(*it->second); return true; }
};
static std::map<const void *, int> g_param_slot; static std::mutex g_param_slot_mu;
static std::atomic<int> g_param_slot_n{ 0 };
static int default_slot() { const int d = g_device.load(std::memory_order_relaxed); return d < 0 ? 0 : d % MAX_SLOTS; }
static int slot_of_graph(const void *g);
static int slot_for(const void *param, const void *g) {
    if (param && g_param_slot_n.load(std::memory_order_acquire) > 0) { std::lock_guard<std::mutex> lk(g_param_slot_mu); auto it = g_param_slot.find(param); if (it != g_param_slot.end()) return it->second; }
    if (!param && g) { const int s = slot_of_graph(g); if (s >= 0) return s; }
    return default_slot();
}
struct SlotLock {
    int slot; std::unique_lock<std::mutex> lk;
    SlotLock(const void *param, const void *g) : slot(slot_for(param, g)), lk(g_slot_mu[slot]) {
        for (int now; (now = slot_for(param, g)) != slot; ) { lk.unlock(); slot = now; lk = std::unique_lock<std::mutex>(g_slot_mu[slot]); }
        t_slot = slot;
        if (device_count() > 0) {
            const int dev = physical_device(slot);
            int cur = -1;
            if (t_device != dev || hipGetDevice(&cur) != hipSuccess || cur != dev) { (void)hipSetDevice(dev); t_device = dev; }
        }
    }
};
static std::once_flag g_dev_once;
static void ensure_device() {
    std::call_once(g_dev_once, [] {
        load_env_options();
        int n = device_count();
        if (n <= 0) fail(ERR_NO_DEVICE, "no HIP device visible: the april_graph_cholesky* / april_graph_chi2 entry points of "
                         "libaprilsam_amd.so run on an AMD GPU only (there is NO CPU fallback: nothing was computed)");
        if (g_device < 0) {
            const char *lr = getenv("LOCAL_RANK");
            g_device = lr ? atoi(lr) % n : 0;
        }
    });
}

template <class T> struct DBuf {
    T *p = nullptr; size_t cap = 0;
    bool need(size_t n) {
// ... 114 lines not shown
        (void)hipGetLastError();
    });
}

int selftest() {
    const int cases[][2] = { { 12, 0 }, { 12, 30 }, { 45, 17 }, { 100, 0 }, { 130, 64 }, { 43, 200 }, { 11, 11 }, { 87, 1 } };
    for (auto &cs : cases) {
        const int nsb = cs[0], nub = cs[1], nbc = nsb + nub, R = 3 * (nbc + 1), C = 3 * nbc, ns = 3 * nsb, Rv = R - 2;
        std::vector<int> applied((size_t)Rv * C, 0);
        std::vector<long long> ksum((size_t)Rv * C, 0);
        const int steps = (ns + NB - 1) / NB;
        auto run = [&](int s_lo, int s_hi, int tile, bool ahead = false) -> int {
            const SyrkRange g = syrk_range(R, C, ns, s_lo, s_hi, tile, ahead);
            const int nt = syrk_tiles(R, C, ns, s_lo, s_hi, tile, ahead);
            if (nt != g.ntc * g.ntr - g.ntc * (g.ntc - 1) / 2) return -11;
            std::vector<char> seen((size_t)std::max(1, g.ntr) * std::max(1, g.ntc), 0);
            for (int l = 0; l < nt; l++) {
                int tj = 0; while (tj + 1 < g.ntc && (tj + 1) * g.ntr - (tj + 1) * tj / 2 <= l) tj++;
                const int ti = tj + (l - (tj * g.ntr - tj * (tj - 1) / 2));
                if (ti < tj || ti >= g.ntr || seen[(size_t)tj * g.ntr + ti]++) return -12;
                for (int j = g.col_lo + tj * tile; j < std::min(g.col_hi, g.col_lo + (tj + 1) * tile); j++)
                    for (int i = std::max(j, g.col_lo + ti * tile); i < std::min(Rv, g.col_lo + (ti + 1) * tile); i++)
                        for (int k = g.k_lo; k < g.k_hi; k++) { applied[(size_t)j * Rv + i]++; ksum[(size_t)j * Rv + i] += k; }
            }
            return 0;
        };
        for (int tile : { TILE, TILE / 2 }) {
            std::fill(applied.begin(), applied.end(), 0); std::fill(ksum.begin(), ksum.end(), 0);
            for (int o = 0; o * OBP < steps; o++) {
                const int k0 = o * OBP * NB, k1 = std::min(ns, k0 + OBP * NB);
                for (int j = k0; j < k1; j++)
                    for (int i = j; i < Rv; i++)
                        if (applied[(size_t)j * Rv + i] != k0 || ksum[(size_t)j * Rv + i] != (long long)k0 * (k0 - 1) / 2) return -13;
                const int rc = run(o * OBP, (o + 1) * OBP, tile); if (rc) return rc;
            }
            for (int j = ns; j < C; j++)
                for (int i = j; i < Rv; i++)
                    if (applied[(size_t)j * Rv + i] != ns || ksum[(size_t)j * Rv + i] != (long long)ns * (ns - 1) / 2) return -14;
        }
        for (int G : { 2, 3, 4 }) for (int tile : { TILE, TILE / 2 }) {
            std::fill(applied.begin(), applied.end(), 0); std::fill(ksum.begin(), ksum.end(), 0);
            const int nobs = (steps + OBP - 1) / OBP;
            for (int o = 0; o < nobs; o++) {
                const int k0 = o * OBP * NB, k1 = std::min(ns, k0 + OBP * NB);
                for (int j = k0; j < k1; j++)
                    for (int i = j; i < Rv; i++)
                        if (applied[(size_t)j * Rv + i] != k0 || ksum[(size_t)j * Rv + i] != (long long)k0 * (k0 - 1) / 2) return -15;
                int rc;
                const int g0 = (o - o % G) * OBP;
                if (o % G != G - 1) rc = run(g0, (o + 1) * OBP, tile, o + 1 < nobs);
                else rc = run(g0, (o + 1) * OBP, tile);
                if (rc) return rc;
            }
            for (int j = ns; j < C; j++)
                for (int i = j; i < Rv; i++)
                    if (applied[(size_t)j * Rv + i] != ns || ksum[(size_t)j * Rv + i] != (long long)ns * (ns - 1) / 2) return -16;
        }
        long long run_off = 0;
        for (int j = ns; j < C; j++) { if (upd_packed_offset(R, ns, j) != run_off) return -21; run_off += Rv - 3 * (j / 3); }
        if (upd_packed_offset(R, ns, C) != run_off) return -22;
        for (int o = 0; o * OBP < steps; o++)
            for (int rb : { 1, 2 }) {
                const int c1 = std::min(ns, (o + 1) * OBW), below = Rv - c1, nt = block_tiles(R, ns, o, rb);
                if ((long long)nt * BLOCK_ROWS * rb < below || (nt > 0 && (long long)(nt - 1) * BLOCK_ROWS * rb >= below)) return -31;
            }
    }
    for (int ntr = 1; ntr <= 75; ntr += (ntr < 20 ? 1 : 7))
        for (int ntc = 1; ntc <= ntr; ntc += (ntc < 20 ? 1 : 5)) {
            const int nt = ntc * ntr - ntc * (ntc - 1) / 2;
            std::vector<char> seen((size_t)ntr * ntc, 0);
            for (int l = 0; l < nt; l++) {
                int ti = -1, tj = -1;
                trapezoid_tile_xcd(l, nt, ntr, ntc, &ti, &tj);
                if (tj < 0 || tj >= ntc || ti < tj || ti >= ntr || seen[(size_t)tj * ntr + ti]++) return -35;
            }
        }
    for (int nw : { 4, 8, 16 })
        for (int R = 6; R < 400; R += 7)
            for (int nsb = 1; 3 * nsb < R - 3; nsb += 5) {
                const int C = R - 3;
                if (panel_front_lds(R, 3 * nsb, nw) > small_front_lds(R, C, nw)) return -41;
                if (small_front_lds(R, C, nw) != (size_t)(R | 1) * C * 8 + (size_t)wl_bytes(nw)) return -42;
            }
    return 0;
}

int api_device_count() { return device_count(); }
int api_set_device(int d) {
    int n = device_count();
    if (d < 0 || d >= n) return -1;
    g_device = d;
    return 0;
}
int api_param_set_device(const april_graph_cholesky_param_t *param, int slot) {
    if (!param || slot < 0 || slot >= MAX_SLOTS) return -1;
    { SlotLock lk0(param, nullptr); drop_shard_state(param); }
    drop_context(param);
    std::lock_guard<std::mutex> lk(g_param_slot_mu);
    g_param_slot[param] = slot;
    g_param_slot_n.store((int)g_param_slot.size(), std::memory_order_release);
    return 0;
}
int api_param_get_device(const april_graph_cholesky_param_t *param) { return physical_device(slot_for(param, nullptr)); }
void unbind_param(const april_graph_cholesky_param_t *param) {
    if (g_param_slot_n.load(std::memory_order_acquire) == 0) return;
    std::lock_guard<std::mutex> lk(g_param_slot_mu);
    g_param_slot.erase(param);
    g_param_slot_n.store((int)g_param_slot.size(), std::memory_order_release);
}
int api_set_option(const char *name, double v) {
    load_env_options();
    const OptionDef *d = name ? find_option(name) : nullptr;
    if (!d) return -1;
    const int nv = std::min(d->max_value, std::max(d->min_value, (int)v));
    if (g_opt.*(d->member) == nv) return 0;
    g_opt.*(d->member) = nv;
    if (!d->policy) g_opt_epoch++;
    return 0;
}
int api_get_option(const char *name, double *v) {
    load_env_options();
    const OptionDef *d = name ? find_option(name) : nullptr;
    if (!d || !v) return -1;
    *v = (double)(g_opt.*(d->member));
    return 0;
}

}

extern "C" int aprilsam_amd_marginals(april_graph_t *graph, april_graph_cholesky_param_t *param, int n, const int *nodes, double *cov) {
    return asam::marginals(graph, param, n, nodes, nullptr, cov, false);
}
extern "C" int aprilsam_amd_marginals_joint(april_graph_t *graph, april_graph_cholesky_param_t *param, int n, const int *a, const int *b, double *cov) {
    return asam::marginals(graph, param, n, a, b, cov, true);
}
extern "C" int aprilsam_amd_max_selected(april_graph_t *graph, april_graph_cholesky_param_t *param, int n, const int *factors, int *out) {
    return asam::max_selected(graph, param, n, factors, out);
}
extern "C" int aprilsam_amd_robust_weights(april_graph_t *graph, april_graph_cholesky_param_t *param, int n, const int *factors, double *w) {
    return asam::robust_weights(graph, param, n, factors, w);
}
extern "C" long long aprilsam_amd_debug_selinv_runs(const april_graph_cholesky_param_t *param) { return asam::selinv_runs(param); }
extern "C" int aprilsam_amd_marginals_joint_any(april_graph_t *graph, april_graph_cholesky_param_t *param, int n, const int *a, const int *b, double *cov) {
    return asam::marginals_joint_any(graph, param, n, a, b, cov);
}
extern "C" int aprilsam_amd_gate_xyt(april_graph_t *graph, april_graph_cholesky_param_t *param, int n, const int *a, const int *b, const double *z,
                                     const double *W, double *d2, double *S) {
    return asam::gate_xyt(graph, param, n, a, b, z, W, d2, S);
}
extern "C" long long aprilsam_amd_debug_path_solve_bytes(const april_graph_cholesky_param_t *param) { return asam::path_solve_bytes(param); }
extern "C" void aprilsam_amd_lm_opts_init(aprilsam_amd_lm_opts_t *opts) { asam::lm_opts_init(opts); }
extern "C" int aprilsam_amd_optimize_lm(april_graph_t *graph, april_graph_cholesky_param_t *param, const aprilsam_amd_lm_opts_t *opts,
                                        aprilsam_amd_lm_report_t *report, double *trace) {
    return asam::optimize_lm(graph, param, opts, report, trace);
}
```

### aprilsam_amd/csrc/solver_context.inc.h

```cpp
enum { K_LINEARIZE = 0, K_FRONT_SMALL, K_ASSEMBLE_BIG, K_PANEL_BIG, K_SYRK_BIG, K_BACKSOLVE, K_UPDATE, NKERN };
static const char *const KNAMES[NKERN] = { "k_linearize", "k_front_small", "k_assemble_big", "k_panel_big", "k_syrk_big", "k_backsolve", "k_update_states" };
struct Launch { int list_off, pre_off, n, grid; bool single = false; int tile = TILE; };

struct LevelPlan {
    int small_off = 0, n_small = 0; size_t small_lds = 0;
    long long full_limit = 0;
    int small_nt = 512;
    int n_big = 0; size_t asm_lds = 0;
    Launch asm_big{};
    std::vector<Launch> syrka, syrk1;
    bool paired = false;
    std::vector<Launch> bchain, btile, syrkw;
    int all_off = 0, n_all = 0; size_t solve_lds = 0;
    size_t solve_w_lds = 0; int maxns = 0;
    Launch bs_gemv{};
    Launch bs_blk{}; size_t bs_blk_lds = 0;
    int rest_off = 0, n_rest = 0; size_t rest_lds = 0;
};

struct IncState {
    bool ready = false;
    bool pristine = false;
    int Nb = 0, Fb = 0, nF0 = 0, nLev0 = 0;
    int cap_nodes = 0, cap_fact = 0;
// ... 7 lines not shown
    std::vector<int> bf_ptr, bf_idx;
    std::vector<int> rel_begin;
    std::vector<int> cur_nub;
    std::vector<long long> cur_cap;
    std::vector<char> dirty;
    std::vector<int> f_level;
    int zpos = 0;
    int tail_ok = -1;
    int recs_stale = -1;
    std::vector<int> t_first, t_cnt;
    std::vector<int> tf_of;
    std::vector<std::vector<int>> kids;
    std::vector<LevelPlan> base_levels;
    std::vector<int> st_i32, st_tab, st_sb, st_sr, st_ids; std::vector<DestRec> st_dest; std::vector<ChildRec> st_child;
    std::vector<unsigned char> st_sw; std::vector<double> st_zeros; std::vector<char> need;
    std::vector<char> stale;
    bool upd_ok = true;
    bool base_has_big = false;
    std::vector<char> st_mid, st_mode; std::vector<int> st_owner, st_mask, st_wout, st_slot; std::vector<UpdRec> st_upd, st_rec;
};

struct SelLevel { int gat_off = 0, n_gat = 0, diag_off = 0, n_diag = 0, tri_off = 0, n_tri = 0, x_off = 0, n_x = 0, sus_off = 0, n_sus = 0, sss_off = 0, n_sss = 0; };

struct PathState {
    long long serial = -1;
    int N = 0;
    std::vector<SelFront> fr; std::vector<int> depth, i32, rec, node_j;
    DBuf<PsFront> d_fr; DBuf<int4> d_ent; DBuf<int> d_cmap; DBuf<long long> d_at; DBuf<PsPath> d_path; DBuf<PsPair> d_pair;
    DBuf<double> d_buf, d_cov, d_in; HBuf<double> h_out;
    long long peak_doubles = 0;
    void release() {
        d_fr.release(); d_ent.release(); d_cmap.release(); d_at.release(); d_path.release(); d_pair.release(); d_buf.release(); d_cov.release(); d_in.release(); h_out.release();
        fr.clear(); depth.clear(); i32.clear(); rec.clear(); node_j.clear(); serial = -1;
    }
};

struct Context {
    Plan plan;
    bool have_plan = false;
    std::vector<int> pat;
    int patN = 0;
    DBuf<int> d_i32; DBuf<FrontDesc> d_fd; DBuf<DestRec> d_dest; DBuf<ChildRec> d_child; DBuf<double> d_lambda;
    DevPlan dp{};
    DBuf<int> d_tab;
    std::vector<LevelPlan> levels;
    DBuf<unsigned char> d_swap;
    DBuf<int> d_pos;
    DBuf<long long> d_prof;
    DBuf<double> d_pool, d_H, d_x, d_diag;
    DBuf<int> d_bad;
    HBuf<int> h_bad;
    IncPrologue pro{}; InlinePatches inl{};
    bool no_speculation = false;
    HBuf<long long> h_kstamp; HBuf<int> h_done; int done_seq = 0, one_wait = 0;
    std::vector<double> h_lambda;
    aprilsam_amd_stats_t st{};
    hipEvent_t ev[8] = {};
    bool have_events = false;
    double k_ms[NKERN] = {}; long long k_calls[NKERN] = {};
    std::vector<hipEvent_t> k_ev; std::vector<int> k_ids, k_lev;
    std::vector<double> lev_up_ms, lev_dn_ms;
    bool have_fact = false;
    int plan_pin = 0;
    long long plan_persist = 0;
    int same_topo_batches = 0;
    bool used_inc = false;
    bool want_inc = false;
    int batch_nodes = 0;
    IncState inc;
    int inc_F = 0, inc_N = 0;
    std::vector<RefModel::Visit> visits; std::vector<int> involved;
    std::vector<int> base_tab;
    std::vector<int> inc_slot_blk, inc_slot_rhs;
    long long pat_serial = -1, pat_topo = -1;
    RefModel model;
    PatchList patches;
    int batch_factors = 0;
    std::vector<unsigned char> wt; bool wt_any = false, wt_dirty = false;
    long long wt_serial = -1, wt_topo = -1, wt_content = -1;
    DBuf<long long> d_guard; DBuf<int> d_guard_cnt; int n_guard = 0, guard_len = 0;
    std::vector<unsigned char> swap_host;
    int persist_l0 = -1;
    int p_up_off = 0, p_up_n = 0, p_dn_off = 0, p_dn_n = 0, p_nt = 1024; size_t p_up_lds = 0, p_dn_lds = 0; long long p_up_full = 0; int p_dn_maxns = 0;
    DBuf<int> d_flags, d_flevel, d_perm, d_epoch, d_marks;
    int flag_stride = 0;
    long long epoch_steps = 0;
    DBuf<double> d_dinv, d_bsb_far; DBuf<int> d_bsb_flags;
    DBuf<int> d_solve_tab; std::vector<int> solve_tab;
    DBuf<UpdRec> d_upd; DBuf<double> d_wbuf;
    hipGraphExec_t gexec = nullptr;
    const void *gexec_key = nullptr;
    long long gexec_serial = 0;
    long long gexec_mx = -1;
    long long gexec_rb = -1;
    hipGraphExec_t gexec_api = nullptr;
    const void *api_key[9] = {};
    hipGraphExec_t gexec_lm = nullptr;
    const void *lm_key[9] = {};
    DBuf<double> d_lm_trial, d_lm_hacc, d_lm_terms, d_lm_trace; DBuf<LmScalars> d_lm; HBuf<LmScalars> h_lm;
    int api_key_runs = 0;
    struct Retired { hipGraphExec_t g; hipEvent_t done; };
    std::vector<Retired> retired;
    hipStream_t graph_stream = nullptr;
    void reap_retired(bool wait = false) {
        size_t keep = 0;
        for (Retired &r : retired) {
            if (r.done) {
                if (wait) (void)hipEventSynchronize(r.done);
                else if (hipEventQuery(r.done) != hipSuccess) { retired[keep++] = r; continue; }
                (void)hipEventDestroy(r.done);
            }
            (void)hipGraphExecDestroy(r.g);
        }
        retired.resize(keep);
    }
    void retire(hipGraphExec_t &g) {
        if (!g) return;
        if (retired.size() >= 8) reap_retired();
        if (retired.size() >= 32) reap_retired(true);
        Retired r{ g, nullptr };
        if (graph_stream && hipEventCreateWithFlags(&r.done, hipEventDisableTiming) == hipSuccess) {
            if (hipEventRecord(r.done, graph_stream) != hipSuccess) { (void)hipEventDestroy(r.done); r.done = nullptr; }
        } else r.done = nullptr;
        retired.push_back(r); g = nullptr;
    }
    double lambda_val = -1; int lambda_N = -1;
    int fact_kind = 0; long long fact_epoch = -1; bool fact_asym = false;
    DBuf<double> d_sigma, d_sel_scr; DBuf<SelFront> d_sel_fd; DBuf<int> d_sel_i32, d_sel_q; DBuf<int4> d_sel_ent; HBuf<double> h_cov;
    long long fact_serial = 0;
    std::vector<SelLevel> sel_levels; int sel_tab_kind = 0, sel_N = 0;
    long long sel_serial = -1, sel_tab_serial = -1, sel_runs = 0, sel_pool = 1; double sel_flops = 0;
    PathState ps;
    void release_sel() {
        d_sigma.release(); d_sel_scr.release(); d_sel_fd.release(); d_sel_i32.release(); d_sel_q.release(); d_sel_ent.release(); h_cov.release();
        sel_levels.clear(); sel_serial = -1; sel_tab_serial = -1;
        ps.release();
    }
    void release() {
        release_sel();
        d_i32.release(); d_fd.release(); d_dest.release(); d_child.release(); d_lambda.release(); d_tab.release(); d_swap.release(); d_pos.release();
        d_pool.release(); d_H.release(); d_x.release(); d_diag.release(); d_bad.release(); h_bad.release(); patches.release();
        h_done.release(); h_kstamp.release(); d_prof.release(); d_upd.release(); d_wbuf.release(); d_flags.release(); d_flevel.release(); d_epoch.release(); d_marks.release(); d_perm.release(); d_solve_tab.release(); d_dinv.release(); d_bsb_far.release(); d_bsb_flags.release(); d_guard.release(); d_guard_cnt.release(); n_guard = 0;
        d_lm_trial.release(); d_lm_hacc.release(); d_lm_terms.release(); d_lm_trace.release(); d_lm.release(); h_lm.release();
        retire(gexec); retire(gexec_api); retire(gexec_lm); reap_retired(true);
        if (have_events) for (auto &e : ev) (void)hipEventDestroy(e);
        have_events = false;
        for (auto &e : k_ev) (void)hipEventDestroy(e);
        k_ev.clear();
    }
};
static Registry<Context> g_ctx;

static void forget_stream(hipStream_t s) {
    g_ctx.for_each([&](Context &c) { if (c.graph_stream == s) c.graph_stream = nullptr; });
}

static Context &ctx_for(const april_graph_cholesky_param_t *p) {
    auto it = g_ctx.find(p);
    if (it == g_ctx.end()) it = g_ctx.emplace(p, std::make_unique<Context>()).first;
    return *it->second;
}
void drop_context(const april_graph_cholesky_param_t *p) {
    SlotLock lk(p, nullptr);
    auto it = g_ctx.find(p);
    if (it != g_ctx.end()) { it->second->release(); g_ctx.erase(it); }
}
// ... 252 lines not shown
    const double u1 = uprof ? now_ms() : 0;
    const bool inc = c.want_inc;
    const int INC_NODES_ = inc ? INC_NODES : 0, INC_FACT_ = inc ? INC_FACT : 0;
    const size_t INC_I32_ = inc ? INC_I32 : 0, INC_DEST_ = inc ? INC_DEST : 0, INC_CHILD_ = inc ? INC_CHILD : 0, INC_TAB_ = inc ? INC_TAB : 0;
    c.inc.cap_nodes = INC_NODES_; c.inc.cap_fact = INC_FACT_;
    std::vector<int> i32;
    auto put32 = [&](const std::vector<int> &v) { size_t o = i32.size(); i32.insert(i32.end(), v.begin(), v.end()); if (v.empty()) i32.push_back(0); return o; };
    size_t o_rows = put32(P.f_rows), o_rel = put32(P.f_rel);
    size_t o_sb = put32(P.slot_blk); i32.resize(i32.size() + (size_t)3 * INC_FACT_, -1);
    size_t o_sr = put32(P.slot_rhs); i32.resize(i32.size() + (size_t)2 * INC_FACT_, -1);
    c.inc.i32_used = (long long)i32.size(); c.inc.dest_used = (long long)P.dest.size(); c.inc.child_used = (long long)P.ch_idx.size();
    for (int t = 0; t < P.nF; t++) fd[t].rows_begin = (int)(o_rows + P.f_rows_ptr[t]);
    for (size_t k = 0; k < P.ch_idx.size(); k++) ch[k].rel_begin = (int)(o_rel + P.f_rows_ptr[ch[k].pad]);
    c.d_i32.need(i32.size() + INC_I32_); c.d_fd.need(fd.size() + 1 + (inc ? MAX_TAIL_FRONTS : 0)); c.d_child.need(ch.size() + INC_CHILD_);
    c.d_dest.need(std::max<size_t>(1, P.dest.size()) + INC_DEST_);
    HIPCHECK(hipMemcpyAsync(c.d_i32.p, i32.data(), i32.size() * 4, hipMemcpyHostToDevice, s));
    HIPCHECK(hipMemcpyAsync(c.d_fd.p, fd.data(), fd.size() * sizeof(FrontDesc), hipMemcpyHostToDevice, s));
    HIPCHECK(hipMemcpyAsync(c.d_child.p, ch.data(), ch.size() * sizeof(ChildRec), hipMemcpyHostToDevice, s));
    static_assert(sizeof(DestRec) == sizeof(Plan::DestRec), "DestRec layout");
    if (!P.dest.empty()) HIPCHECK(hipMemcpyAsync(c.d_dest.p, P.dest.data(), P.dest.size() * sizeof(DestRec), hipMemcpyHostToDevice, s));
    c.d_lambda.need((size_t)P.N + INC_NODES_);
    DevPlan &d = c.dp;
    d.nF = P.nF;
    d.fd = c.d_fd.p; d.dest = c.d_dest.p; d.child = c.d_child.p;
    d.f_rows = c.d_i32.p; d.f_rel = c.d_i32.p; d.slot_blk = c.d_i32.p + o_sb; d.slot_rhs = c.d_i32.p + o_sr; d.src_idx = c.d_i32.p;
    c.inc.o_rows = (long long)o_rows; c.inc.o_rel = (long long)o_rel;
    d.lambda = c.d_lambda.p;
    d.prof = nullptr; d.prof_mode = 0;
    d.schur_first_nub = std::max(0, g_opt.schur_first);
    d.epoch = nullptr; d.flevel = nullptr; d.l0 = 0; d.marks = nullptr;
    if (getenv("APRILSAM_AMD_KPROF")) { c.d_prof.need((size_t)PROF_SLOTS * P.nF); HIPCHECK(hipMemsetAsync(c.d_prof.p, 0, (size_t)8 * PROF_SLOTS * P.nF, s)); d.prof = c.d_prof.p; d.prof_mode = atoi(getenv("APRILSAM_AMD_KPROF")) >= 2 ? atoi(getenv("APRILSAM_AMD_KPROF")) : 1; }
    c.d_swap.need((size_t)P.F + INC_FACT_); c.d_pos.need((size_t)P.N + INC_NODES_);
    fill_swap_host(c);
    HIPCHECK(hipMemcpyAsync(c.d_swap.p, c.swap_host.data(), P.F, hipMemcpyHostToDevice, s));
    c.wt_dirty = false;
    HIPCHECK(hipMemcpyAsync(c.d_pos.p, P.pos.data(), (size_t)P.N * 4, hipMemcpyHostToDevice, s));
    c.d_perm.need((size_t)P.N + INC_NODES_);
    HIPCHECK(hipMemcpyAsync(c.d_perm.p, P.perm.data(), (size_t)P.N * 4, hipMemcpyHostToDevice, s));

    const double u2 = uprof ? now_ms() : 0;
    std::vector<int> tab;
    c.levels.assign(P.nLevels, LevelPlan());
    for (int l = 0; l < P.nLevels; l++) {
        std::vector<int> fr(P.lev_fronts.begin() + P.lev_ptr[l], P.lev_fronts.begin() + P.lev_ptr[l + 1]);
        build_level(c.levels[l], fr, tab, [&](int t, int *nsb, int *nub) { *nsb = P.f_nsb[t]; *nub = P.f_nub[t]; }, [](int) { return true; });
    }
    {
        long long slots = 0;
        for (int t = 0; t < P.nF; t++) fd[t].dinv0 = -1;
        for (int l = 0; l < P.nLevels; l++) {
            const LevelPlan &L = c.levels[l];
            for (int k = 0; k < L.asm_big.n; k++) { const int t = tab[L.asm_big.list_off + k]; fd[t].dinv0 = (int)slots; slots += (long long)OBP * bsb_blocks(3 * P.f_nsb[t]); }
        }
        c.d_dinv.need((size_t)std::max<long long>(slots, 1) * NB * NB);
        HIPCHECK(hipMemcpyAsync(c.d_fd.p, fd.data(), fd.size() * sizeof(FrontDesc), hipMemcpyHostToDevice, s));
        if (!c.d_bsb_flags.p) { c.d_bsb_flags.need((size_t)BSB_MAX_WGS * 2 * BSB_MAXB); HIPCHECK(hipMemsetAsync(c.d_bsb_flags.p, 0, c.d_bsb_flags.cap * 4, s)); c.d_bsb_far.need((size_t)BSB_MAX_WGS * BSB_FAR); }
    }
    for (int l = 0; l < P.nLevels; l++)
        if (c.levels[l].solve_lds > 160 * 1024)
            fail(ERR_UNSUPPORTED, "a frontal matrix has more rows than the back-substitution kernel can hold in LDS (an unsplittable dense region "
                 "of more than ~6000 poses); this build does not tile the solve of such a front");
    c.persist_l0 = -1;
    if (g_opt.persist && !lay && P.nLevels >= 3) {
        int l0 = P.nLevels, cnt = 0;
        const int nt_top = c.levels[P.nLevels - 1].small_nt;
        for (int l = P.nLevels - 1; l >= 0; l--) {
            const LevelPlan &L = c.levels[l];
            if (L.n_big > 0 || L.bs_gemv.grid > 0 || L.small_nt != nt_top || L.n_small != L.n_all || cnt + L.n_small > g_opt.persist_max_fronts) break;
            cnt += L.n_small; l0 = l;
        }
        if (P.nLevels - l0 >= 2) {
            c.persist_l0 = l0; c.p_nt = nt_top; c.p_up_lds = 0; c.p_dn_lds = 0; c.p_up_full = 0; c.p_dn_maxns = 0;
            c.p_up_off = (int)tab.size(); c.p_up_n = cnt;
            for (int l = l0; l < P.nLevels; l++) {
                const LevelPlan &L = c.levels[l];
                for (int k = 0; k < L.n_small; k++) tab.push_back(tab[L.small_off + k]);
                c.p_up_lds = std::max(c.p_up_lds, L.small_lds); c.p_up_full = std::max(c.p_up_full, L.full_limit);
                for (int k = 0; k < L.n_all; k++) { const int t = tab[L.all_off + k]; c.p_dn_lds = std::max(c.p_dn_lds, backsolve_lds(P.cols(t), 3 * P.f_nsb[t], true)); c.p_dn_maxns = std::max(c.p_dn_maxns, 3 * P.f_nsb[t]); }
            }
            c.p_dn_off = (int)tab.size(); c.p_dn_n = cnt;
            for (int l = P.nLevels - 1; l >= l0; l--) { const LevelPlan &L = c.levels[l]; for (int k = 0; k < L.n_all; k++) tab.push_back(tab[L.all_off + k]); }
        }
    }
    {
        const size_t stride = (size_t)P.nF + MAX_TAIL_FRONTS;
        const bool fresh = c.d_flags.need(3 * stride);
        c.d_flevel.need(stride);
        if (fresh || (size_t)c.flag_stride != stride) HIPCHECK(hipMemsetAsync(c.d_flags.p, 0, c.d_flags.cap * 4, s));
        c.flag_stride = (int)stride;
        if (c.d_marks.need(stride)) HIPCHECK(hipMemsetAsync(c.d_marks.p, 0, c.d_marks.cap * 4, s));
        if (c.d_epoch.need(1)) { HIPCHECK(hipMemcpyAsync(c.d_epoch.p, &FIRST_EPOCH, 4, hipMemcpyHostToDevice, s)); c.epoch_steps = 0; }
        d.epoch = c.d_epoch.p;
    }
    if (inc) { c.d_upd.need((size_t)g_opt.persist_max_fronts + 64); c.d_wbuf.need((size_t)1 << 19); }
    HIPCHECK(hipMemcpyAsync(c.d_flevel.p, P.f_level.data(), (size_t)P.nF * 4, hipMemcpyHostToDevice, s));
    if (tab.empty()) tab.push_back(0);
    c.d_tab.need(tab.size() + INC_TAB_);
    c.inc.tab_used = (long long)tab.size();
    c.base_tab = tab;
    const double u3 = uprof ? now_ms() : 0;
    HIPCHECK(hipMemcpyAsync(c.d_tab.p, tab.data(), tab.size() * 4, hipMemcpyHostToDevice, s));
    HIPCHECK(hipStreamSynchronize(s));
    const double u4 = uprof ? now_ms() : 0;

    const long long pool_slack = inc ? std::max<long long>(INC_POOL_MIN, P.pool_doubles / 4) : 0;
    const long long pool_doubles = lay ? lay->pool_doubles : P.pool_doubles;
    c.d_pool.need((size_t)std::max<long long>(pool_doubles, 1) + (size_t)pool_slack);
    c.inc.pool_used = pool_doubles; c.inc.pool_cap = (long long)c.d_pool.cap;
    c.n_guard = 0;
    if (g_opt.pool_guard > 0 && !lay) {
        const long long G = ((long long)g_opt.pool_guard + 31) & ~31ll;
        std::vector<long long> go((size_t)P.nF);
        for (int t = 0; t < P.nF; t++) go[t] = P.f_off[t] + ((((long long)P.rows(t) * P.cols(t)) + 31) & ~31ll);
        c.d_guard.need((size_t)P.nF); c.d_guard_cnt.need(2);
        HIPCHECK(hipMemcpyAsync(c.d_guard.p, go.data(), go.size() * 8, hipMemcpyHostToDevice, s));
        HIPCHECK(hipMemsetAsync(c.d_guard_cnt.p, 0, 8, s));
        c.n_guard = P.nF; c.guard_len = (int)G;
        hipLaunchKernelGGL(k_guard, dim3(c.n_guard), dim3(TPB), 0, s, 0, c.d_guard.p, c.n_guard, c.guard_len, c.d_pool.p, c.d_guard_cnt.p);
        HIPCHECK(hipStreamSynchronize(s));
    }
    c.d_H.need((size_t)9 * ((size_t)std::max(1, P.n_slots) + (size_t)5 * INC_FACT_)); c.d_x.need((size_t)3 * ((size_t)P.N + INC_NODES_ + 1));
    c.inc.zpos = P.N + INC_NODES_;
    HIPCHECK(hipMemsetAsync(c.d_x.p + (size_t)3 * c.inc.zpos, 0, 24, s));
    c.inc.slots_used = P.n_slots;
    c.inc.ready = false; c.inc.t_first.clear(); c.same_topo_batches = 0;
    c.d_bad.need(4); c.h_bad.need(4);
    {
        size_t mx = inc ? diag_doubles(160) : 1;
        for (int l = 0; l < P.nLevels; l++) mx = std::max(mx, diag_doubles(c.levels[l].n_big));
        c.d_diag.need(mx);
    }
    if (uprof) fprintf(stderr, "aprilsam_amd upload: graphs destroyed + descriptors %.3f, index arrays + copies %.3f, launch tables %.3f, last copies + sync %.3f, pools %.3f ms\n", u1 - u0, u2 - u1, u3 - u2, u4 - u3, now_ms() - u4);
    c.st.n_fronts = P.nF; c.st.n_levels = P.nLevels; c.st.max_front_rows = P.max_rows;
    c.st.nnz_L = P.nnzL; c.st.flops_factor = P.flops; c.st.bytes_fronts = 8.0 * (double)pool_doubles;
}

static void set_small_attr() {
    static std::once_flag once[MAX_SLOTS];
    std::call_once(once[physical_device(t_slot) % MAX_SLOTS], [] {
        HIPCHECK(hipFuncSetAttribute((const void *)k_front_small<256>, hipFuncAttributeMaxDynamicSharedMemorySize, 160 * 1024));
        HIPCHECK(hipFuncSetAttribute((const void *)k_front_small<512>, hipFuncAttributeMaxDynamicSharedMemorySize, 160 * 1024));
        HIPCHECK(hipFuncSetAttribute((const void *)k_front_small<1024>, hipFuncAttributeMaxDynamicSharedMemorySize, 160 * 1024));
        HIPCHECK(hipFuncSetAttribute((const void *)k_backsolve_t<false>, hipFuncAttributeMaxDynamicSharedMemorySize, 160 * 1024));
        HIPCHECK(hipFuncSetAttribute((const void *)k_backsolve_t<true>, hipFuncAttributeMaxDynamicSharedMemorySize, 160 * 1024));
        HIPCHECK(hipFuncSetAttribute((const void *)k_backsolve_w, hipFuncAttributeMaxDynamicSharedMemorySize, 160 * 1024));
        HIPCHECK(hipFuncSetAttribute((const void *)k_backsolve_t<false, true>, hipFuncAttributeMaxDynamicSharedMemorySize, 160 * 1024));
        HIPCHECK(hipFuncSetAttribute((const void *)k_block_chain, hipFuncAttributeMaxDynamicSharedMemorySize, 160 * 1024));
        HIPCHECK(hipFuncSetAttribute((const void *)k_backsolve_blk, hipFuncAttributeMaxDynamicSharedMemorySize, 160 * 1024));
        HIPCHECK(hipFuncSetAttribute((const void *)k_block_solve<1>, hipFuncAttributeMaxDynamicSharedMemorySize, 160 * 1024));
        HIPCHECK(hipFuncSetAttribute((const void *)k_block_solve<2>, hipFuncAttributeMaxDynamicSharedMemorySize, 160 * 1024));
        HIPCHECK(hipFuncSetAttribute((const void *)k_inc_one<256>, hipFuncAttributeMaxDynamicSharedMemorySize, 160 * 1024));
        HIPCHECK(hipFuncSetAttribute((const void *)k_inc_one<512>, hipFuncAttributeMaxDynamicSharedMemorySize, 160 * 1024));
        HIPCHECK(hipFuncSetAttribute((const void *)k_inc_one<1024>, hipFuncAttributeMaxDynamicSharedMemorySize, 160 * 1024));
    });
}

template <class Tic, class Toc>
static void launch_backsolve(Context &c, const LevelPlan &L, hipStream_t s, Tic tic, Toc toc, const int *tab = nullptr, UpdArgs upd = UpdArgs{}) {
    if (!tab) tab = c.d_tab.p;
    if (!L.n_all) return;
    tic(K_BACKSOLVE);
    if (L.bs_gemv.grid > 0)
        hipLaunchKernelGGL(k_backsolve_gemv, dim3(L.bs_gemv.grid), dim3(TPB), 0, s, c.dp, tab + L.bs_gemv.list_off, tab + L.bs_gemv.pre_off,
                           L.bs_gemv.n, c.d_pool.p, c.d_x.p);
    int n_all = L.n_all, all_off = L.all_off; size_t solve_lds = L.solve_lds;
    if (L.bs_blk.grid > 0) {
        hipLaunchKernelGGL(k_backsolve_blk, dim3(L.bs_blk.grid), dim3(TPB), L.bs_blk_lds, s, c.dp, tab + L.bs_blk.list_off, tab + L.bs_blk.pre_off, L.bs_blk.n,
                           c.d_pool.p, c.d_x.p, c.d_dinv.p, c.d_bsb_flags.p, c.d_bsb_far.p, L.bs_gemv.grid > 0 ? 1 : 0, c.d_bad.p, upd);
        n_all = L.n_rest; all_off = L.rest_off; solve_lds = L.rest_lds;
        if (!n_all) { toc(); return; }
    }
    if (g_opt.wave_backsolve && L.bs_gemv.grid == 0 && L.n_all < g_opt.tp_fronts && L.maxns <= BSW_MAX_NS && L.solve_w_lds <= 80 * 1024)
        hipLaunchKernelGGL(k_backsolve_w, dim3(n_all), dim3(TPB), L.solve_w_lds, s, c.dp, tab + all_off, c.d_pool.p, c.d_x.p, (int *)nullptr, c.d_bad.p, upd);
    else if (solve_lds >= (size_t)(BS_TALL_ROWS + NB + 8 + NB * (NB + 1)) * 8)
        hipLaunchKernelGGL((k_backsolve_t<false, true>), dim3(n_all), dim3(TPB), solve_lds, s, c.dp, tab + all_off, c.d_pool.p, c.d_x.p, L.bs_gemv.grid > 0 ? 1 : 0, (int *)nullptr, 0, c.d_bad.p, upd);
    else
        hipLaunchKernelGGL((k_backsolve_t<false>), dim3(n_all), dim3(TPB), solve_lds, s, c.dp, tab + all_off, c.d_pool.p, c.d_x.p, L.bs_gemv.grid > 0 ? 1 : 0, (int *)nullptr, 0, c.d_bad.p, upd);
    toc();
}

static DevPlan persist_plan(const Context &c) { DevPlan d = c.dp; d.flevel = c.d_flevel.p; d.l0 = c.persist_l0; return d; }
static void rewind_epoch(Context &c, hipStream_t s, long long phases) {
    c.epoch_steps += phases;
    if (c.epoch_steps < (1ll << 30) || !c.d_epoch.p) return;
    c.fact_kind = FACT_NONE;
    HIPCHECK(hipStreamSynchronize(s));
    HIPCHECK(hipMemsetAsync(c.d_flags.p, 0, c.d_flags.cap * 4, s));
    HIPCHECK(hipMemsetAsync(c.d_marks.p, 0, c.d_marks.cap * 4, s));
    HIPCHECK(hipMemcpyAsync(c.d_epoch.p, &FIRST_EPOCH, 4, hipMemcpyHostToDevice, s));
    c.epoch_steps = phases;
}
static void enqueue_poison(Context &c, hipStream_t s, const int *list, int n, int what = 3, const UpdRec *recs = nullptr) {
    if (g_opt.pool_poison <= 0 || n <= 0) return;
    static_assert(offsetof(UpdRec, mode) % 4 == 0 && sizeof(UpdRec) % 4 == 0, "UpdRec::mode as a strided int");
    hipLaunchKernelGGL(k_poison, dim3(n), dim3(TPB), 0, s, c.dp, list, n, recs ? (const int *)((const char *)recs + offsetof(UpdRec, mode)) : (const int *)nullptr,
                       (int)(sizeof(UpdRec) / 4), what, c.d_pool.p, c.d_x.p);
}
static void launch_front_persist(Context &c, hipStream_t s) {
    const int *list = c.d_tab.p + c.p_up_off;
    int *fl = c.d_flags.p;
    DevPlan dpe = persist_plan(c);
    if (g_opt.skip_flag_waits > 0) dpe.l0 = 1 << 30;
    if (c.p_nt >= 1024) hipLaunchKernelGGL(k_front_small<1024>, dim3(c.p_up_n), dim3(1024), c.p_up_lds, s, dpe, list, c.d_pool.p, c.d_H.p, c.d_bad.p, c.p_up_full, fl, 1);
    else if (c.p_nt >= 512) hipLaunchKernelGGL(k_front_small<512>, dim3(c.p_up_n), dim3(512), c.p_up_lds, s, dpe, list, c.d_pool.p, c.d_H.p, c.d_bad.p, c.p_up_full, fl, 1);
    else hipLaunchKernelGGL(k_front_small<256>, dim3(c.p_up_n), dim3(256), c.p_up_lds, s, dpe, list, c.d_pool.p, c.d_H.p, c.d_bad.p, c.p_up_full, fl, 1);
}

static void launch_front_small(Context &c, const LevelPlan &L, hipStream_t s, const int *tab = nullptr) {
    if (!tab) tab = c.d_tab.p;
    const int nt = L.small_nt;
    if (nt >= 1024) hipLaunchKernelGGL(k_front_small<1024>, dim3(L.n_small), dim3(1024), L.small_lds, s, c.dp, tab + L.small_off, c.d_pool.p, c.d_H.p, c.d_bad.p, L.full_limit, (int *)nullptr, 0);
    else if (nt >= 512) hipLaunchKernelGGL(k_front_small<512>, dim3(L.n_small), dim3(512), L.small_lds, s, c.dp, tab + L.small_off, c.d_pool.p, c.d_H.p, c.d_bad.p, L.full_limit, (int *)nullptr, 0);
    else hipLaunchKernelGGL(k_front_small<256>, dim3(L.n_small), dim3(256), L.small_lds, s, c.dp, tab + L.small_off, c.d_pool.p, c.d_H.p, c.d_bad.p, L.full_limit, (int *)nullptr, 0);
}

template <class Tic, class Toc>
static void enqueue_big_steps(Context &c, const LevelPlan &L, hipStream_t s, Tic tic, Toc toc, const int *tab = nullptr) {
    if (!tab) tab = c.d_tab.p;
    const int xcd = std::max(0, g_opt.syrk_xcd_order) << SYRK_MODE_XCD_SHIFT;
    for (size_t o = 0; o < L.bchain.size(); o++) {
        const Launch &bc = L.bchain[o], &bt = L.btile[o], &sw = L.syrkw[o];
        tic(K_PANEL_BIG);
        hipLaunchKernelGGL(k_block_chain, dim3(bc.n), dim3(BCH_THREADS), block_chain_lds(), s, c.dp, tab + bc.list_off, (int)o, c.d_pool.p, c.d_diag.p, c.d_dinv.p, c.d_bad.p);
        if (bt.grid > 0) {
            if (bt.tile == 2) hipLaunchKernelGGL(k_block_solve<2>, dim3(bt.grid), dim3(TPB), block_solve_lds(), s, c.dp, tab + bt.list_off, tab + bt.pre_off, bt.n, (int)o, c.d_pool.p, c.d_diag.p, c.d_dinv.p);
            else hipLaunchKernelGGL(k_block_solve<1>, dim3(bt.grid), dim3(TPB), block_solve_lds(), s, c.dp, tab + bt.list_off, tab + bt.pre_off, bt.n, (int)o, c.d_pool.p, c.d_diag.p, c.d_dinv.p);
        }
        toc();
        auto wide = [&](const Launch &w, int s_lo, int s_hi, int mode) {
            if (w.grid <= 0) return;
            tic(K_SYRK_BIG);
            if (w.tile == TILE / 2) hipLaunchKernelGGL(k_syrk_big32, dim3(w.grid), dim3(TPB), 0, s, c.dp, tab + w.list_off, tab + w.pre_off, w.n, s_lo, s_hi, mode | xcd, c.d_pool.p);
            else hipLaunchKernelGGL(k_syrk_big, dim3(w.grid), dim3(TPB), 0, s, c.dp, tab + w.list_off, tab + w.pre_off, w.n, s_lo, s_hi, mode | xcd, c.d_pool.p);
            toc();
        };
        const int G = std::max(2, g_opt.syrk_group), g0 = (int)(o - o % G) * OBP;
        if (!L.paired) wide(sw, (int)o * OBP, (int)(o + 1) * OBP, 1);
        else if ((int)(o % G) != G - 1) { wide(L.syrka[o], g0, (int)(o + 1) * OBP, 2); wide(L.syrk1[o], g0, (int)(o + 1) * OBP, 1); }
        else wide(sw, g0, (int)(o + 1) * OBP, 1);
    }
}

template <class Tic, class Toc>
static void enqueue_factor_level(Context &c, const LevelPlan &L, hipStream_t s, Tic tic, Toc toc, const int *tab = nullptr) {
    if (!tab) tab = c.d_tab.p;
    if (L.n_small) {
        tic(K_FRONT_SMALL);
        launch_front_small(c, L, s, tab);
        toc();
    }
    if (L.n_big) {
        tic(K_ASSEMBLE_BIG);
        hipLaunchKernelGGL(k_assemble_big, dim3(L.asm_big.grid), dim3(TPB), L.asm_lds, s, c.dp, tab + L.asm_big.list_off,
                           tab + L.asm_big.pre_off, L.asm_big.n, c.d_pool.p, c.d_H.p);
        toc();
        enqueue_big_steps(c, L, s, tic, toc, tab);
    }
}

static void enqueue_numeric(Context &c, GraphPack &gp, hipStream_t s, hipEvent_t *ev, bool unary_at_lp = false, bool ktime = false, bool io_host = false, bool relin = false,
                            double *st_dest = nullptr) {
    const Plan &P = c.plan;
    const int F = P.F, N = P.N;
    size_t nev = 0;
    if (ktime) { c.k_ids.clear(); c.k_lev.clear(); }
    int cur_level = -1;
    auto tic = [&](int id) {
        if (!ktime) return;
        if (c.k_ev.size() < nev + 2) { c.k_ev.resize(nev + 2); HIPCHECK(hipEventCreate(&c.k_ev[nev])); HIPCHECK(hipEventCreate(&c.k_ev[nev + 1])); }
        HIPCHECK(hipEventRecord(c.k_ev[nev], s));
        c.k_ids.push_back(id); c.k_lev.push_back(cur_level);
    };
    auto toc = [&]() { if (ktime) { HIPCHECK(hipEventRecord(c.k_ev[nev + 1], s)); nev += 2; } };
    if (ev) HIPCHECK(hipEventRecord(ev[0], s));
    if (c.dp.prof) HIPCHECK(hipMemsetAsync(c.d_prof.p, 0, (size_t)8 * PROF_SLOTS * P.nF, s));
    if (io_host) hipLaunchKernelGGL(k_load_states, dim3((3 * N + TPB - 1) / TPB), dim3(TPB), 0, s, 3 * N, gp.h_state.p, gp.d_state.p, gp.d_lp.p);
    enqueue_poison(c, s, nullptr, P.nF);
    tic(K_LINEARIZE);
    enqueue_select(gp, s);
    enqueue_robust(gp, s, unary_at_lp ? gp.d_upt.p : (const double *)nullptr);
    {
        auto launch = [&](auto kern) {
            hipLaunchKernelGGL(kern, dim3((F + TPB - 1) / TPB), dim3(TPB), 0, s, 0, F, (const int *)nullptr, gp.d_fa.p, gp.d_fb.p, gp.d_z.p, gp.d_W.p,
                               gp.d_lp.p, gp.d_state.p, c.d_swap.p, c.dp.slot_blk, c.dp.slot_rhs, c.d_H.p, c.d_bad.p, unary_at_lp ? gp.d_upt.p : (const double *)nullptr, c.d_epoch.p);
        };
        if (F >= g_opt.linearize_staged_min) launch(k_linearize_t<true>); else launch(k_linearize_t<false>);
    }
    if (!gp.host_idx.empty()) {
        const int nh = (int)gp.host_idx.size();
        HIPCHECK(hipMemcpyAsync(gp.d_hostH.p, gp.h_hostH.p, (size_t)33 * 8 * nh, hipMemcpyHostToDevice, s));
        hipLaunchKernelGGL(k_scatter_host, dim3((nh + TPB - 1) / TPB), dim3(TPB), 0, s, nh, gp.d_host_idx.p, gp.d_hostH.p, gp.d_fb.p, c.d_swap.p,
                           c.dp.slot_blk, c.dp.slot_rhs, c.d_H.p);
    }
    toc();
    if (ev) HIPCHECK(hipEventRecord(ev[1], s));
    const int l0 = c.persist_l0 >= 0 ? c.persist_l0 : P.nLevels;
    for (int l = 0; l < l0; l++) { cur_level = l; enqueue_factor_level(c, c.levels[l], s, tic, toc); }
    cur_level = l0;
    if (l0 < P.nLevels) { tic(K_FRONT_SMALL); launch_front_persist(c, s); toc(); }
    if (ev) HIPCHECK(hipEventRecord(ev[2], s));
    UpdArgs upd{ c.d_perm.p, gp.d_lp.p, st_dest ? st_dest : gp.d_state.p, gp.d_dx.p, io_host ? gp.h_lp.p : nullptr, io_host ? gp.h_dx.p : nullptr, nullptr, relin ? gp.d_lp.p : nullptr };
    if (l0 < P.nLevels) {
        UpdArgs u = upd; if (l0 == 0) u.bad_out = io_host ? c.h_bad.p : nullptr;
        tic(K_BACKSOLVE);
        if (g_opt.wave_backsolve && c.p_dn_maxns <= BSW_MAX_NS)
            hipLaunchKernelGGL(k_backsolve_w, dim3(c.p_dn_n), dim3(TPB), c.p_dn_lds, s, persist_plan(c), c.d_tab.p + c.p_dn_off, c.d_pool.p, c.d_x.p, c.d_flags.p + c.flag_stride, c.d_bad.p, u);
        else
            hipLaunchKernelGGL((k_backsolve_t<true>), dim3(c.p_dn_n), dim3(TPB), c.p_dn_lds, s, persist_plan(c), c.d_tab.p + c.p_dn_off, c.d_pool.p, c.d_x.p, 0, c.d_flags.p + c.flag_stride, 1, c.d_bad.p, u);
        toc();
    }
    for (int l = l0 - 1; l >= 0; l--) {
        UpdArgs u = upd; if (l == 0) u.bad_out = io_host ? c.h_bad.p : nullptr;
        cur_level = l;
        launch_backsolve(c, c.levels[l], s, tic, toc, nullptr, u);
    }
    if (ev) HIPCHECK(hipEventRecord(ev[3], s));
    HIPCHECK(hipGetLastError());
}
static void collect_kernel_times(Context &c) {
    for (size_t i = 0; i < c.k_ids.size(); i++) {
        float ms = 0;
        HIPCHECK(hipEventElapsedTime(&ms, c.k_ev[2 * i], c.k_ev[2 * i + 1]));
        c.k_ms[c.k_ids[i]] += ms; c.k_calls[c.k_ids[i]]++;
        const int l = i < c.k_lev.size() ? c.k_lev[i] : -1;
        if (l >= 0) {
            if (c.lev_up_ms.size() <= (size_t)l) { c.lev_up_ms.resize(l + 1, 0.0); c.lev_dn_ms.resize(l + 1, 0.0); }
            (c.k_ids[i] == K_BACKSOLVE ? c.lev_dn_ms : c.lev_up_ms)[l] += ms;
        }
    }
    c.k_ids.clear();
}

static void run_numeric(Context &c, GraphPack &gp, bool timing, bool unary_at_lp = false, bool io_host = false, bool relin = false) {
    hipStream_t s = gp.stream;
    set_small_attr();
    rewind_epoch(c, s, 1);
    if (timing && !c.have_events) { for (auto &e : c.ev) HIPCHECK(hipEventCreate(&e)); c.have_events = true; }
    if (io_host) {
        if (g_opt.use_graph && !timing && gp.host_idx.empty()) {
            const void *key[9] = { gp.d_state.p, gp.h_state.p, gp.h_lp.p, gp.h_dx.p, c.h_bad.p, (const void *)(size_t)gp.N, (const void *)(size_t)gp.serial, (const void *)(size_t)gp.mx_gen,
                                   (const void *)(size_t)gp.rb_gen };
            if (memcmp(key, c.api_key, sizeof(key)) != 0) { c.retire(c.gexec_api); memcpy(c.api_key, key, sizeof(key)); c.api_key_runs = 0; }
            if (c.api_key_runs++ == 0) { enqueue_numeric(c, gp, s, nullptr, false, false, true); return; }
            if (!c.gexec_api) {
                hipGraph_t graph = nullptr;
                HIPCHECK(hipStreamBeginCapture(s, hipStreamCaptureModeThreadLocal));
                enqueue_numeric(c, gp, s, nullptr, false, false, true);
                HIPCHECK(hipStreamEndCapture(s, &graph));
                HIPCHECK(hipGraphInstantiate(&c.gexec_api, graph, nullptr, nullptr, 0));
                HIPCHECK(hipGraphDestroy(graph));
            }
            c.graph_stream = s;
            HIPCHECK(hipGraphLaunch(c.gexec_api, s));
        } else {
            enqueue_numeric(c, gp, s, timing ? c.ev : nullptr, false, false, true);
        }
        return;
    }
    if (g_opt.use_graph && !timing && !unary_at_lp && gp.host_idx.empty()) {
        if (!c.gexec || c.gexec_key != (const void *)gp.d_state.p || c.gexec_serial != gp.serial || c.gexec_mx != gp.mx_gen || c.gexec_rb != gp.rb_gen) {
            c.retire(c.gexec);
            hipGraph_t graph = nullptr;
            HIPCHECK(hipStreamBeginCapture(s, hipStreamCaptureModeThreadLocal));
            enqueue_numeric(c, gp, s, nullptr, false, false, false, relin);
            HIPCHECK(hipStreamEndCapture(s, &graph));
            HIPCHECK(hipGraphInstantiate(&c.gexec, graph, nullptr, nullptr, 0));
            HIPCHECK(hipGraphDestroy(graph));
            c.gexec_key = (const void *)gp.d_state.p; c.gexec_serial = gp.serial; c.gexec_mx = gp.mx_gen; c.gexec_rb = gp.rb_gen;
        }
        c.graph_stream = s;
        HIPCHECK(hipGraphLaunch(c.gexec, s));
    } else {
        enqueue_numeric(c, gp, s, timing ? c.ev : nullptr, unary_at_lp, false, false, relin);
    }
}

static double device_chi2(GraphPack &gp) {
    hipStream_t s = gp.stream;
    if (gp.F == 0) return 0;
    hipLaunchKernelGGL(k_chi2, dim3((gp.F + TPB - 1) / TPB), dim3(TPB), 0, s, gp.F, gp.d_fa.p, gp.d_fb.p, gp.d_z.p, gp.d_W.p, gp.d_state.p, gp.d_chi2f.p);
    enqueue_chi2_mixture(gp, s);
    enqueue_chi2_robust(gp, s);
    if (gp.F > REDUCE_SPLIT) {
        double *parts = gp.d_chi2f.p + gp.F_cap;
        hipLaunchKernelGGL(k_reduce_parts, dim3(REDUCE_PARTS), dim3(TPB), 0, s, gp.F, gp.d_chi2f.p, parts);
        hipLaunchKernelGGL(k_reduce, dim3(1), dim3(1024), 0, s, REDUCE_PARTS, parts, gp.d_scalar.p);
    } else hipLaunchKernelGGL(k_reduce, dim3(1), dim3(1024), 0, s, gp.F, gp.d_chi2f.p, gp.d_scalar.p);
    HIPCHECK(hipMemcpyAsync(gp.h_scalar.p, gp.d_scalar.p, 8, hipMemcpyDeviceToHost, s));
    HIPCHECK(hipStreamSynchronize(s));
    return gp.h_scalar.p[0];
}

static long long g_opt_epoch = 0;
static long long launch_table_key() { return g_opt_epoch; }
static void set_wt_any(Context &c, bool v) { c.wt_any = v; }
static bool orient_asymmetric(Context &c, GraphPack &gp) {
    if (gp.n_asym == 0) {
// ... 55 lines not shown
```

### aprilsam_amd/csrc/symbolic.cpp

```cpp
#include "plan.h"
#include "solver.h"
#include "errors.h"

#include <algorithm>
#include <atomic>
#include <cassert>
#include <cstdio>
#include <cstdlib>
#include <tuple>
#include <chrono>
#include <mutex>

namespace asam {

static void amalgamate(NDTree &tree, int N, const std::vector<int> &ap, const std::vector<int> &ai, int max_own, size_t lds_budget) {
    const double HAND = 12.0 + 2.7, PERCOL = 0.19 + 0.8 / 64.0;
    constexpr int REGION_MAX = 4096;
    const int nT = (int)tree.nodes.size();
    std::vector<int> order; order.reserve(nT);
    {
        std::vector<std::pair<int, size_t>> st;
        for (int r : tree.roots) {
            st.push_back({ r, 0 });
            while (!st.empty()) {
// ... 255 lines not shown
            for (int t = t0; t < t1; t++) {
                int d = P.dest_front_ptr[t] - 1;
                for (int i = ptr[t]; i < ptr[t + 1]; i++) {
                    const unsigned long long k = key[i];
                    const int col = (int)(k >> (1 + KEY_SRC_BITS + KEY_ROW_BITS)), row = (int)((k >> (1 + KEY_SRC_BITS)) & ((1u << KEY_ROW_BITS) - 1)) - 1,
                              src = (int)((k >> 1) & ((1u << KEY_SRC_BITS) - 1)), rhs = (int)(k & 1);
                    if (i == ptr[t] || !same_dest(k, key[i - 1])) P.dest[++d] = { row, col, i, i };
                    P.dest[d].src_end = i + 1;
                    (rhs ? P.slot_rhs : P.slot_blk)[src] = i;
                }
            }
        });
        P.n_slots = (int)total;
    }

    stamp();
    P.f_off.assign(nT, 0);
    int64_t off = 0;
    P.max_rows = 0; P.nnzL = 0; P.flops = 0;
    for (int t = 0; t < nT; t++) {
        P.f_off[t] = off;
        int64_t sz = (int64_t)P.rows(t) * P.cols(t);
        off += (sz + 31) & ~int64_t(31);
        int ns = 3 * P.f_nsb[t], nu = 3 * P.f_nub[t];
        P.max_rows = std::max(P.max_rows, ns + nu);
        P.nnzL += (int64_t)ns * (ns + 1) / 2 + (int64_t)nu * ns;
        for (int q = 0; q < ns; q++) { double c = (double)(ns - q) + nu; P.flops += c * c; }
    }
    P.pool_doubles = off;
    stamp();
    if (prof && nph == 8)
        fprintf(stderr, "aprilsam_amd planner N=%d F=%d: adjacency %.3f dissection %.3f front structure %.3f levels %.3f factor lists %.3f records+slots %.3f offsets %.3f | total %.3f ms\n",
                N, F, tph[1] - tph[0], tph[2] - tph[1], tph[3] - tph[2], tph[4] - tph[3], tph[5] - tph[4], tph[6] - tph[5], tph[7] - tph[6], tph[7] - tph[0]);
}

void build_gather_lists(Plan &P) {
    if (!P.bd_front_ptr.empty()) return;
    const int F = P.F, nT = P.nF;
    struct Dest { int front, col, row, src; };
    std::vector<Dest> bd, rd; bd.reserve((size_t)3 * F); rd.reserve((size_t)2 * F);
    for (int f = 0; f < F; f++) {
        const int t = P.fac_front[f], la = P.fac_la[f], lb = P.fac_lb[f];
        if (t < 0) continue;
        bd.push_back({ t, la, la, 3 * f + 0 });
        rd.push_back({ t, la, 0, 2 * f + 0 });
        if (lb >= 0) {
            bd.push_back({ t, std::min(la, lb), std::max(la, lb), 3 * f + 1 });
            bd.push_back({ t, lb, lb, 3 * f + 2 });
            rd.push_back({ t, lb, 0, 2 * f + 1 });
        }
    }
    auto sort_dests = [&](std::vector<Dest> &v) {
        std::vector<int> ptr(nT + 1, 0);
        for (const Dest &d : v) ptr[d.front + 1]++;
        for (int t = 0; t < nT; t++) ptr[t + 1] += ptr[t];
        std::vector<unsigned long long> key(v.size());
        { std::vector<int> fill(ptr.begin(), ptr.end() - 1);
          for (const Dest &d : v) key[fill[d.front]++] = ((unsigned long long)(unsigned)d.col << 44) | ((unsigned long long)(unsigned)(d.row + 1) << 26) | (unsigned)d.src; }
        for (int t = 0; t < nT; t++) {
            std::sort(key.begin() + ptr[t], key.begin() + ptr[t + 1]);
            for (int i = ptr[t]; i < ptr[t + 1]; i++) v[i] = { t, (int)(key[i] >> 44), (int)((key[i] >> 26) & 0x3ffff) - 1, (int)(key[i] & 0x3ffffff) };
        }
    };
    sort_dests(bd);
    sort_dests(rd);
    auto compress = [&](const std::vector<Dest> &v, std::vector<int> &front_ptr, std::vector<int> &row, std::vector<int> &col,
                        std::vector<int> &src_ptr, std::vector<int> &src) {
        front_ptr.assign(nT + 1, 0); row.clear(); col.clear(); src_ptr.clear(); src.clear();
        src_ptr.push_back(0);
        for (size_t i = 0; i < v.size(); i++) {
            bool fresh = i == 0 || v[i].front != v[i - 1].front || v[i].col != v[i - 1].col || v[i].row != v[i - 1].row;
            if (fresh) { if (i) src_ptr.push_back((int)src.size()); row.push_back(v[i].row); col.push_back(v[i].col); front_ptr[v[i].front + 1]++; }
            src.push_back(v[i].src);
        }
        if (!v.empty()) src_ptr.push_back((int)src.size());
        for (int t = 0; t < nT; t++) front_ptr[t + 1] += front_ptr[t];
    };
    std::vector<int> dummy_row;
    compress(bd, P.bd_front_ptr, P.bd_row, P.bd_col, P.bd_src_ptr, P.bd_src);
    compress(rd, P.rd_front_ptr, dummy_row, P.rd_col, P.rd_src_ptr, P.rd_src);
}

}
```

### include/aprilsam_amd.h

```cpp
#ifndef APRILSAM_AMD_H
#define APRILSAM_AMD_H

#include <stddef.h>
#include <stdint.h>

#ifdef __cplusplus
extern "C" {
#endif


typedef struct zarray {
    size_t el_sz;
    int    size;
    int    alloc;
    char  *data;
} zarray_t;

typedef struct matd {
    unsigned int nrows, ncols;
    double       data[];
} matd_t;

typedef struct april_graph {
    zarray_t   *factors;
// ... 140 lines not shown
int  aprilsam_amd_last_error(char *msg, int cap);
void aprilsam_amd_clear_error(void);

int aprilsam_amd_set_option(const char *name, double value);
int aprilsam_amd_debug_guard_selftest(const april_graph_cholesky_param_t *param);
int aprilsam_amd_get_option(const char *name, double *value);

int aprilsam_amd_batch_resident(april_graph_t *graph, april_graph_cholesky_param_t *param, int iters,
                                double *chi2_out, double *ms_out);

int    aprilsam_amd_resident_begin(april_graph_t *graph, april_graph_cholesky_param_t *param);
int    aprilsam_amd_resident_steps(april_graph_t *graph, april_graph_cholesky_param_t *param, int n, int mode);
int    aprilsam_amd_resident_sync(april_graph_t *graph, april_graph_cholesky_param_t *param);
double aprilsam_amd_resident_chi2(april_graph_t *graph);
int    aprilsam_amd_resident_end(april_graph_t *graph, april_graph_cholesky_param_t *param);
int aprilsam_amd_kernel_profile(const april_graph_cholesky_param_t *param, double *ms, long long *calls,
                                double *flops, double *bytes, const char **names);
int aprilsam_amd_level_profile(const april_graph_cholesky_param_t *param, double *out6, int cap_levels);

int aprilsam_amd_marginals(april_graph_t *graph, april_graph_cholesky_param_t *param, int n, const int *nodes, double *cov);
int aprilsam_amd_marginals_joint(april_graph_t *graph, april_graph_cholesky_param_t *param, int n, const int *a, const int *b, double *cov);
long long aprilsam_amd_debug_selinv_runs(const april_graph_cholesky_param_t *param);

int aprilsam_amd_marginals_joint_any(april_graph_t *graph, april_graph_cholesky_param_t *param, int n, const int *a, const int *b, double *cov);
int aprilsam_amd_gate_xyt(april_graph_t *graph, april_graph_cholesky_param_t *param, int n, const int *a, const int *b, const double *z,
                          const double *W, double *d2, double *S);
long long aprilsam_amd_debug_path_solve_bytes(const april_graph_cholesky_param_t *param);

typedef struct {
    int    max_iters;
    int    check_every;
    double lambda0;
    double lambda_max;
    double eta;
    double ftol;
    double xtol;
} aprilsam_amd_lm_opts_t;
void aprilsam_amd_lm_opts_init(aprilsam_amd_lm_opts_t *opts);

enum { APRILSAM_AMD_LM_CONVERGED_F = 1, APRILSAM_AMD_LM_CONVERGED_X = 2, APRILSAM_AMD_LM_STALLED = 3, APRILSAM_AMD_LM_MAX_ITERS = 4 };
typedef struct {
    int    status, iterations, accepted, rejected_not_spd;
    double F_initial, F_final;
    double chi2_final;
    double lambda_final;
} aprilsam_amd_lm_report_t;

int aprilsam_amd_optimize_lm(april_graph_t *graph, april_graph_cholesky_param_t *param, const aprilsam_amd_lm_opts_t *opts,
                             aprilsam_amd_lm_report_t *report, double *trace);

#define APRILSAM_AMD_FACTOR_MAX_TYPE 3
april_graph_factor_t *aprilsam_amd_factor_max_create(april_graph_factor_t **components, const double *logw, int n);
int aprilsam_amd_max_selected(april_graph_t *graph, april_graph_cholesky_param_t *param, int n, const int *factors, int *out);

enum { APRILSAM_AMD_ROBUST_NONE = 0, APRILSAM_AMD_ROBUST_HUBER = 1, APRILSAM_AMD_ROBUST_CAUCHY = 2, APRILSAM_AMD_ROBUST_DCS = 3 };
int aprilsam_amd_factor_set_robust(april_graph_factor_t *factor, int kind, double c);
int aprilsam_amd_factor_get_robust(const april_graph_factor_t *factor, int *kind, double *c);
int aprilsam_amd_robust_weights(april_graph_t *graph, april_graph_cholesky_param_t *param, int n, const int *factors, double *w);

typedef struct aprilsam_amd_host_comm {
    void *user;
    int (*send)(void *user, const double *buf, long long count, int dst);
    int (*recv)(void *user, double *buf, long long count, int src);
    int (*bcast)(void *user, double *buf, long long count, int root);
    int (*allreduce_sum)(void *user, double *buf, long long count);
} aprilsam_amd_host_comm_t;
int       aprilsam_amd_shard_begin(april_graph_t *graph, april_graph_cholesky_param_t *param, int rank, int world);
long long aprilsam_amd_shard_info(const april_graph_cholesky_param_t *param, int what, long long *out, long long cap);
int       aprilsam_amd_shard_comm_unique_id(char *out128);
int       aprilsam_amd_shard_comm_init_rccl(april_graph_cholesky_param_t *param, const char *id128);
int       aprilsam_amd_shard_comm_init_host(april_graph_cholesky_param_t *param, const aprilsam_amd_host_comm_t *callbacks);
int       aprilsam_amd_shard_comm_info(const april_graph_cholesky_param_t *param, long long *out5, char *rccl_path, int cap);
int       aprilsam_amd_shard_iterate(april_graph_t *graph, april_graph_cholesky_param_t *param, int n);
int       aprilsam_amd_shard_gather_states(april_graph_t *graph, april_graph_cholesky_param_t *param);
double    aprilsam_amd_shard_chi2(april_graph_t *graph, april_graph_cholesky_param_t *param);
void      aprilsam_amd_shard_end(april_graph_cholesky_param_t *param);

typedef struct aprilsam_amd_plan aprilsam_amd_plan_t;
aprilsam_amd_plan_t *aprilsam_amd_plan_create(int n_nodes, int n_factors, const int *factor_nodes ,
                                              const double *xy , int leaf_nodes);
void aprilsam_amd_plan_destroy(aprilsam_amd_plan_t *plan);
long long aprilsam_amd_plan_query(const aprilsam_amd_plan_t *plan, const char *what, long long **out);
long long aprilsam_amd_shard_plan(const aprilsam_amd_plan_t *plan, int world, int what, long long *out, long long cap);
void aprilsam_amd_free(void *p);

int aprilsam_amd_reference_order(int n_nodes, int n_factors, const int *fa, const int *fb, int *out_order, int *out_parent);

void *aprilsam_amd_refmodel_create(void);
void  aprilsam_amd_refmodel_destroy(void *m);
void  aprilsam_amd_refmodel_batch(void *m, int n_nodes, int n_factors, const int *fa, const int *fb);
int   aprilsam_amd_refmodel_inc_begin(void *m, int n_nodes, int n_factors, const int *fa, const int *fb);
int   aprilsam_amd_refmodel_solve_visit(void *m, const double *x, double dxy, double dth, int *visited);
void  aprilsam_amd_refmodel_get(void *m, int *parent, int *changed, int *relin);
int   aprilsam_amd_refmodel_check(void *m);

int aprilsam_amd_make_lattice(april_graph_t *graph, int K);
int aprilsam_amd_lattice_arrays(int K, double *states, int *fa, int *fb, double *z, double *W);
void aprilsam_amd_graph_from_arrays(april_graph_t *graph, int N, const double *states, int F, const int *fa,
                                    const int *fb, const double *z, const double *W);

void aprilsam_amd_graph_node_arrays(const april_graph_t *graph, double *state, double *l_point, double *delta_X);

int aprilsam_amd_debug_stage(april_graph_t *graph, april_graph_cholesky_param_t *param, int what, double *out);

int aprilsam_amd_debug_front_times(const april_graph_cholesky_param_t *param, long long *out, int n_fronts);

const char *aprilsam_amd_version(void);

#ifdef __cplusplus
}
#endif
#endif
```

Before: 4685 GN iterations/s.

## Place persistent front blocks so parent-child chains share an XCD

Adds an XCD-aware placement pass. It splits the elimination tree into heavy-path chains and assigns each chain to one of 8 XCD classes, assuming workgroups are dispatched round-robin by block index modulo 8. The persistent upward factor list, the downward backsolve list and the leaf level are then reordered and padded with -1 slots so that a child and its parent run on the same XCD. Kernels skip padded slots. The aim is to keep front data in the local L2 shared by a parent and its children and to cut cross-XCD flag and cache traffic. The cost is extra empty blocks and a dependence on the hardware dispatch order, which is not guaranteed.

```diff
diff --git a/aprilsam_amd/csrc/capi.cpp b/aprilsam_amd/csrc/capi.cpp
--- a/aprilsam_amd/csrc/capi.cpp
+++ b/aprilsam_amd/csrc/capi.cpp
@@ -1,3 +1,4 @@
+#include <algorithm>
 #include <cstdio>
 #include <cstdlib>
 #include <cstring>
@@ -143,6 +144,20 @@
     else if (what == 4) v = asam::shard_critical_path(plan->P, world, owner, top); else return -1;
     if (out) for (long long i = 0; i < (long long)v.size() && i < cap; i++) out[i] = v[i];
     return (long long)v.size();
+}
+
+int aprilsam_amd_xcd_place(int nF, const int *parent, const int *level, const int *nsb, int l0, int cap, int cap_leaf, int which, int *out, int out_cap) {
+    if (nF < 0 || !parent || !level || !nsb || which < 0 || which > 3) return -100;
+    std::vector<int> up, leaves;
+    int top = 0;
+    for (int t = 0; t < nF; t++) top = std::max(top, level[t]);
+    for (int l = l0; l <= top; l++) for (int t = 0; t < nF; t++) if (level[t] == l) up.push_back(t);
+    if (l0 == 1) for (int t = 0; t < nF; t++) if (level[t] == 0) leaves.push_back(t);
+    const asam::XcdLists x = asam::xcd_place(up, leaves, parent, nsb, nF, cap, cap_leaf);
+    if (which == 3) return asam::xcd_check(x, up, leaves, parent, nF, cap, cap_leaf);
+    const std::vector<int> &v = which == 0 ? x.up : which == 1 ? x.dn : x.leaf;
+    if (out) for (int i = 0; i < (int)v.size() && i < out_cap; i++) out[i] = v[i];
+    return (int)v.size();
 }
 
 long long aprilsam_amd_plan_query(const aprilsam_amd_plan_t *plan, const char *what, long long **out) {
diff --git a/aprilsam_amd/csrc/kernels.hip.h b/aprilsam_amd/csrc/kernels.hip.h
--- a/aprilsam_amd/csrc/kernels.hip.h
+++ b/aprilsam_amd/csrc/kernels.hip.h
@@ -6,6 +6,8 @@
 namespace asam {
 
 constexpr int PROF_SLOTS = 16;
+constexpr int PROF_XCD_UP = 12, PROF_XCD_DN = 13;
+__device__ __forceinline__ int xcc_id() { return __builtin_amdgcn_s_getreg(20 | (0 << 6) | ((4 - 1) << 11)) & 7; }
 constexpr int TPB = 256;
 constexpr int NB = 32;
 constexpr int TILE = 64;
@@ -907,6 +909,7 @@
     const int nsb = D.nsb, nbc = D.nsb + D.nub;
     const int R = 3 * (nbc + 1), C = 3 * nbc, ld = R | 1;
     double *Fg = pool + D.off;
+    if (P.prof && threadIdx.x == 0) P.prof[(size_t)t * PROF_SLOTS + PROF_XCD_UP] = 1 + xcc_id();
     if ((long long)small_front_lds(R, C, NT / 64) <= full_lds_limit) {
         int2 *wl = (int2 *)(S + (size_t)ld * C);
         if (P.prof && threadIdx.x == 0) P.prof[(size_t)t * PROF_SLOTS + 0] = wall_clock64();
@@ -1243,11 +1246,13 @@
                                                     const double *__restrict__ Hc, int *bad, long long full_lds_limit,
                                                     int *flags = nullptr, int wait = 0, UpdCtx uc = UpdCtx{}) {
     extern __shared__ __attribute__((aligned(16))) double S[];
+    const int t = fronts[blockIdx.x];
+    if (t < 0) return;
     if (uc.recs) {
         const UpdRec *rec = uc.recs + blockIdx.x;
-        if (rec->mode) { front_update_body<NT>(P, fronts[blockIdx.x], *rec, uc, pool, flags, bad, S); return; }
-    }
-    front_small_body<NT>(P, fronts[blockIdx.x], pool, Hc, bad, full_lds_limit, flags, wait, S);
+        if (rec->mode) { front_update_body<NT>(P, t, *rec, uc, pool, flags, bad, S); return; }
+    }
+    front_small_body<NT>(P, t, pool, Hc, bad, full_lds_limit, flags, wait, S);
 }
 
 constexpr int ASM_INV_CAP = 4096;
@@ -1807,6 +1812,7 @@
                                                      double *__restrict__ x, int split, int *xflags, int wait, int *bad, UpdArgs upd) {
     extern __shared__ __attribute__((aligned(16))) double smem[];
     const int t = fronts[blockIdx.x];
+    if (t < 0) return;
     const int ev = xflags ? flag_value(P) : 0;
     const FrontDesc D_ = P.fd[t];
     const int nsb = D_.nsb, nub = D_.nub, nbc = nsb + nub;
@@ -2131,6 +2137,7 @@
     const int tid = threadIdx.x, wave = tid >> 6, lane = tid & 63;
     const int *rows = P.f_rows + D_.rows_begin;
     long long *pf = (P.prof && P.prof_mode == 2) ? P.prof + (size_t)t * PROF_SLOTS : nullptr;
+    if (pf && tid == 0) pf[PROF_XCD_DN] = 1 + xcc_id();
     {
         const int ne = ns * R;
         for (int e0 = tid; e0 < ne; e0 += 8 * TPB) {
@@ -2202,7 +2209,9 @@
 __global__ void __launch_bounds__(TPB) k_backsolve_w(DevPlan P, const int *__restrict__ fronts, const double *__restrict__ pool,
                                                      double *__restrict__ x, int *xflags, int *bad, UpdArgs upd) {
     extern __shared__ __attribute__((aligned(16))) double smem[];
-    backsolve_w_body(P, fronts[blockIdx.x], pool, x, xflags, bad, upd, smem);
+    const int t = fronts[blockIdx.x];
+    if (t < 0) return;
+    backsolve_w_body(P, t, pool, x, xflags, bad, upd, smem);
 }
 
 __host__ __device__ inline long long upd_packed_offset(int R, int ns, int j) {
diff --git a/aprilsam_amd/csrc/plan.h b/aprilsam_amd/csrc/plan.h
--- a/aprilsam_amd/csrc/plan.h
+++ b/aprilsam_amd/csrc/plan.h
@@ -58,6 +58,10 @@
 void build_plan(Plan &P, int N, int F, const int *factor_nodes, const double *xy, int leaf_nodes);
 void build_gather_lists(Plan &P);
 
+struct XcdLists { std::vector<int> up, dn, leaf; };
+XcdLists xcd_place(const std::vector<int> &up, const std::vector<int> &leaves, const int *parent, const int *nsb, int nF, int cap, int cap_leaf);
+int xcd_check(const XcdLists &x, const std::vector<int> &up, const std::vector<int> &leaves, const int *parent, int nF, int cap, int cap_leaf);
+
 struct NDTree {
     struct Node { std::vector<int> verts; std::vector<int> children; };
     std::vector<Node> nodes;
diff --git a/aprilsam_amd/csrc/solver.h b/aprilsam_amd/csrc/solver.h
--- a/aprilsam_amd/csrc/solver.h
+++ b/aprilsam_amd/csrc/solver.h
@@ -39,6 +39,7 @@
     int extend_tail_fronts = 3;
     int persist = 1;
     int persist_max_fronts = 240;
+    int xcd_place = 1;
     int tail_poses = 28;
     int blk_backsolve = 1;
     int wave_backsolve = 1;
diff --git a/aprilsam_amd/csrc/solver.hip.cpp b/aprilsam_amd/csrc/solver.hip.cpp
--- a/aprilsam_amd/csrc/solver.hip.cpp
+++ b/aprilsam_amd/csrc/solver.hip.cpp
@@ -59,7 +59,7 @@
     { "inc_inline", &Options::inc_inline, 0, true }, { "inc_update", &Options::inc_update, 0, true }, { "inc_tail_solve", &Options::inc_tail_solve, 0, true },
     { "inc_lazy_states", &Options::inc_lazy_states, 0, true }, { "inc_replan_tall", &Options::inc_replan_tall, 0, true },
     { "speculate_factors", &Options::speculate_factors, 0, true }, { "warm_up", &Options::warm_up, 0, true }, { "pin_last", &Options::pin_last, 0, false }, { "persist", &Options::persist, 0, false },
-    { "persist_max_fronts", &Options::persist_max_fronts, 0, false }, { "linearize_staged_min", &Options::linearize_staged_min, 0, false },
+    { "persist_max_fronts", &Options::persist_max_fronts, 0, false }, { "xcd_place", &Options::xcd_place, 0, false }, { "linearize_staged_min", &Options::linearize_staged_min, 0, false },
     { "wave_backsolve", &Options::wave_backsolve, 0, false }, { "blk_backsolve", &Options::blk_backsolve, 0, false }, { "tail_poses", &Options::tail_poses, 8, false },
     { "batch_extend", &Options::batch_extend, 0, true }, { "extend_tail_fronts", &Options::extend_tail_fronts, 0, true }, { "mem_cap_mb", &Options::mem_cap_mb, 0, true },
     { "pool_guard", &Options::pool_guard, 0, false }, { "amalg", &Options::amalg, 0, false }, { "amalg_max", &Options::amalg_max, 1, false }, { "pool_poison", &Options::pool_poison, 0, false }, { "skip_flag_waits", &Options::skip_flag_waits, 0, false },
@@ -340,6 +340,30 @@
                 if (panel_front_lds(R, 3 * nsb, nw) > small_front_lds(R, C, nw)) return -41;
                 if (small_front_lds(R, C, nw) != (size_t)(R | 1) * C * 8 + (size_t)wl_bytes(nw)) return -42;
             }
+    for (int kind = 0; kind < 3; kind++)
+        for (int cap : { 2, 8, 32 }) {
+            const int nF = kind == 2 ? 150 : 400;
+            std::vector<int> parent(nF, -1), nsb(nF), level(nF, 0);
+            unsigned r = 12345u + 77u * kind + (unsigned)cap;
+            auto rnd = [&](int m) { r = r * 1103515245u + 12345u; return (int)((r >> 8) % (unsigned)m); };
+            for (int t = 0; t < nF - 1; t++) {
+                if (kind == 0) parent[t] = t + 1 + rnd(std::min(20, nF - 1 - t));
+                else if (kind == 1) parent[t] = t % 3 == 0 ? t + 1 : std::min(nF - 1, t + 3 - t % 3);
+                else parent[t] = nF - 1;
+                nsb[t] = 1 + rnd(30);
+            }
+            nsb[nF - 1] = 12;
+            for (int t = 0; t < nF - 1; t++) level[parent[t]] = std::max(level[parent[t]], level[t] + 1);
+            int top = 0; for (int t = 0; t < nF; t++) top = std::max(top, level[t]);
+            for (int l0 : { 0, 1, 2 }) {
+                std::vector<int> up, leaves;
+                for (int l = l0; l <= top; l++) for (int t = 0; t < nF; t++) if (level[t] == l) up.push_back(t);
+                if (l0 == 1) for (int t = 0; t < nF; t++) if (level[t] == 0) leaves.push_back(t);
+                const XcdLists x = xcd_place(up, leaves, parent.data(), nsb.data(), nF, cap, cap);
+                const int rc = xcd_check(x, up, leaves, parent.data(), nF, cap, cap);
+                if (rc) return -50 + rc;
+            }
+        }
     return 0;
 }
 
diff --git a/aprilsam_amd/csrc/solver_context.inc.h b/aprilsam_amd/csrc/solver_context.inc.h
--- a/aprilsam_amd/csrc/solver_context.inc.h
+++ b/aprilsam_amd/csrc/solver_context.inc.h
@@ -113,6 +113,8 @@
     std::vector<unsigned char> swap_host;
     int persist_l0 = -1;
     int p_up_off = 0, p_up_n = 0, p_dn_off = 0, p_dn_n = 0, p_nt = 1024; size_t p_up_lds = 0, p_dn_lds = 0; long long p_up_full = 0; int p_dn_maxns = 0;
+    int x_up_off = 0, x_up_n = 0, x_dn_off = 0, x_dn_n = 0;
+    int x_leaf_off = 0, x_leaf_n = 0;
     DBuf<int> d_flags, d_flevel, d_perm, d_epoch, d_marks;
     int flag_stride = 0;
     long long epoch_steps = 0;
@@ -531,6 +533,22 @@
             for (int l = P.nLevels - 1; l >= l0; l--) { const LevelPlan &L = c.levels[l]; for (int k = 0; k < L.n_all; k++) tab.push_back(tab[L.all_off + k]); }
         }
     }
+    c.x_up_n = c.x_dn_n = c.x_leaf_n = 0;
+    if (c.persist_l0 >= 0 && g_opt.xcd_place) {
+        int cus = 0;
+        HIPCHECK(hipDeviceGetAttribute(&cus, hipDeviceAttributeMultiprocessorCount, physical_device(t_slot)));
+        const int per_xcd = std::max(1, cus / 8);
+        auto per_cu = [](size_t lds, int nt) { return std::max(1, std::min(2048 / std::max(nt, 64), (int)((160 * 1024) / std::max<size_t>(lds, 1)))); };
+        const std::vector<int> up(tab.begin() + c.p_up_off, tab.begin() + c.p_up_off + c.p_up_n);
+        const LevelPlan &L0 = c.levels[0];
+        const bool leaf = c.persist_l0 == 1 && L0.n_big == 0 && L0.bs_gemv.grid == 0 && L0.bs_blk.grid == 0 && L0.n_small == L0.n_all;
+        const std::vector<int> leaves = leaf ? std::vector<int>(tab.begin() + L0.small_off, tab.begin() + L0.small_off + L0.n_small) : std::vector<int>();
+        const int cap = per_xcd * per_cu(c.p_up_lds, c.p_nt), cap_leaf = per_xcd * (((int)leaves.size() + 8 * per_xcd - 1) / (8 * per_xcd));
+        const XcdLists x = xcd_place(up, leaves, P.f_parent.data(), P.f_nsb.data(), P.nF, cap, cap_leaf);
+        c.x_up_off = (int)tab.size(); c.x_up_n = (int)x.up.size(); tab.insert(tab.end(), x.up.begin(), x.up.end());
+        c.x_dn_off = (int)tab.size(); c.x_dn_n = (int)x.dn.size(); tab.insert(tab.end(), x.dn.begin(), x.dn.end());
+        c.x_leaf_off = (int)tab.size(); c.x_leaf_n = (int)x.leaf.size(); tab.insert(tab.end(), x.leaf.begin(), x.leaf.end());
+    }
     {
         const size_t stride = (size_t)P.nF + MAX_TAIL_FRONTS;
         const bool fresh = c.d_flags.need(3 * stride);
@@ -605,14 +623,14 @@
 }
 
 template <class Tic, class Toc>
-static void launch_backsolve(Context &c, const LevelPlan &L, hipStream_t s, Tic tic, Toc toc, const int *tab = nullptr, UpdArgs upd = UpdArgs{}) {
+static void launch_backsolve(Context &c, const LevelPlan &L, hipStream_t s, Tic tic, Toc toc, const int *tab = nullptr, UpdArgs upd = UpdArgs{}, int list_off = -1, int list_n = 0) {
     if (!tab) tab = c.d_tab.p;
     if (!L.n_all) return;
     tic(K_BACKSOLVE);
     if (L.bs_gemv.grid > 0)
         hipLaunchKernelGGL(k_backsolve_gemv, dim3(L.bs_gemv.grid), dim3(TPB), 0, s, c.dp, tab + L.bs_gemv.list_off, tab + L.bs_gemv.pre_off,
                            L.bs_gemv.n, c.d_pool.p, c.d_x.p);
-    int n_all = L.n_all, all_off = L.all_off; size_t solve_lds = L.solve_lds;
+    int n_all = list_off >= 0 ? list_n : L.n_all, all_off = list_off >= 0 ? list_off : L.all_off; size_t solve_lds = L.solve_lds;
     if (L.bs_blk.grid > 0) {
         hipLaunchKernelGGL(k_backsolve_blk, dim3(L.bs_blk.grid), dim3(TPB), L.bs_blk_lds, s, c.dp, tab + L.bs_blk.list_off, tab + L.bs_blk.pre_off, L.bs_blk.n,
                            c.d_pool.p, c.d_x.p, c.d_dinv.p, c.d_bsb_flags.p, c.d_bsb_far.p, L.bs_gemv.grid > 0 ? 1 : 0, c.d_bad.p, upd);
@@ -646,21 +664,22 @@
                        (int)(sizeof(UpdRec) / 4), what, c.d_pool.p, c.d_x.p);
 }
 static void launch_front_persist(Context &c, hipStream_t s) {
-    const int *list = c.d_tab.p + c.p_up_off;
+    const bool xp = c.x_up_n > 0;
+    const int *list = c.d_tab.p + (xp ? c.x_up_off : c.p_up_off), n = xp ? c.x_up_n : c.p_up_n;
     int *fl = c.d_flags.p;
     DevPlan dpe = persist_plan(c);
     if (g_opt.skip_flag_waits > 0) dpe.l0 = 1 << 30;
-    if (c.p_nt >= 1024) hipLaunchKernelGGL(k_front_small<1024>, dim3(c.p_up_n), dim3(1024), c.p_up_lds, s, dpe, list, c.d_pool.p, c.d_H.p, c.d_bad.p, c.p_up_full, fl, 1);
-    else if (c.p_nt >= 512) hipLaunchKernelGGL(k_front_small<512>, dim3(c.p_up_n), dim3(512), c.p_up_lds, s, dpe, list, c.d_pool.p, c.d_H.p, c.d_bad.p, c.p_up_full, fl, 1);
-    else hipLaunchKernelGGL(k_front_small<256>, dim3(c.p_up_n), dim3(256), c.p_up_lds, s, dpe, list, c.d_pool.p, c.d_H.p, c.d_bad.p, c.p_up_full, fl, 1);
-}
-
-static void launch_front_small(Context &c, const LevelPlan &L, hipStream_t s, const int *tab = nullptr) {
+    if (c.p_nt >= 1024) hipLaunchKernelGGL(k_front_small<1024>, dim3(n), dim3(1024), c.p_up_lds, s, dpe, list, c.d_pool.p, c.d_H.p, c.d_bad.p, c.p_up_full, fl, 1);
+    else if (c.p_nt >= 512) hipLaunchKernelGGL(k_front_small<512>, dim3(n), dim3(512), c.p_up_lds, s, dpe, list, c.d_pool.p, c.d_H.p, c.d_bad.p, c.p_up_full, fl, 1);
+    else hipLaunchKernelGGL(k_front_small<256>, dim3(n), dim3(256), c.p_up_lds, s, dpe, list, c.d_pool.p, c.d_H.p, c.d_bad.p, c.p_up_full, fl, 1);
+}
+
+static void launch_front_small(Context &c, const LevelPlan &L, hipStream_t s, const int *tab = nullptr, int list_off = -1, int list_n = 0) {
     if (!tab) tab = c.d_tab.p;
-    const int nt = L.small_nt;
-    if (nt >= 1024) hipLaunchKernelGGL(k_front_small<1024>, dim3(L.n_small), dim3(1024), L.small_lds, s, c.dp, tab + L.small_off, c.d_pool.p, c.d_H.p, c.d_bad.p, L.full_limit, (int *)nullptr, 0);
-    else if (nt >= 512) hipLaunchKernelGGL(k_front_small<512>, dim3(L.n_small), dim3(512), L.small_lds, s, c.dp, tab + L.small_off, c.d_pool.p, c.d_H.p, c.d_bad.p, L.full_limit, (int *)nullptr, 0);
-    else hipLaunchKernelGGL(k_front_small<256>, dim3(L.n_small), dim3(256), L.small_lds, s, c.dp, tab + L.small_off, c.d_pool.p, c.d_H.p, c.d_bad.p, L.full_limit, (int *)nullptr, 0);
+    const int nt = L.small_nt, off = list_off >= 0 ? list_off : L.small_off, n = list_off >= 0 ? list_n : L.n_small;
+    if (nt >= 1024) hipLaunchKernelGGL(k_front_small<1024>, dim3(n), dim3(1024), L.small_lds, s, c.dp, tab + off, c.d_pool.p, c.d_H.p, c.d_bad.p, L.full_limit, (int *)nullptr, 0);
+    else if (nt >= 512) hipLaunchKernelGGL(k_front_small<512>, dim3(n), dim3(512), L.small_lds, s, c.dp, tab + off, c.d_pool.p, c.d_H.p, c.d_bad.p, L.full_limit, (int *)nullptr, 0);
+    else hipLaunchKernelGGL(k_front_small<256>, dim3(n), dim3(256), L.small_lds, s, c.dp, tab + off, c.d_pool.p, c.d_H.p, c.d_bad.p, L.full_limit, (int *)nullptr, 0);
 }
 
 template <class Tic, class Toc>
@@ -744,7 +763,11 @@
     toc();
     if (ev) HIPCHECK(hipEventRecord(ev[1], s));
     const int l0 = c.persist_l0 >= 0 ? c.persist_l0 : P.nLevels;
-    for (int l = 0; l < l0; l++) { cur_level = l; enqueue_factor_level(c, c.levels[l], s, tic, toc); }
+    for (int l = 0; l < l0; l++) {
+        cur_level = l;
+        if (l == 0 && c.x_leaf_n > 0) { tic(K_FRONT_SMALL); launch_front_small(c, c.levels[0], s, nullptr, c.x_leaf_off, c.x_leaf_n); toc(); }
+        else enqueue_factor_level(c, c.levels[l], s, tic, toc);
+    }
     cur_level = l0;
     if (l0 < P.nLevels) { tic(K_FRONT_SMALL); launch_front_persist(c, s); toc(); }
     if (ev) HIPCHECK(hipEventRecord(ev[2], s));
@@ -752,16 +775,19 @@
     if (l0 < P.nLevels) {
         UpdArgs u = upd; if (l0 == 0) u.bad_out = io_host ? c.h_bad.p : nullptr;
         tic(K_BACKSOLVE);
+        const bool xp = c.x_dn_n > 0;
+        const int *dn = c.d_tab.p + (xp ? c.x_dn_off : c.p_dn_off), n_dn = xp ? c.x_dn_n : c.p_dn_n;
         if (g_opt.wave_backsolve && c.p_dn_maxns <= BSW_MAX_NS)
-            hipLaunchKernelGGL(k_backsolve_w, dim3(c.p_dn_n), dim3(TPB), c.p_dn_lds, s, persist_plan(c), c.d_tab.p + c.p_dn_off, c.d_pool.p, c.d_x.p, c.d_flags.p + c.flag_stride, c.d_bad.p, u);
+            hipLaunchKernelGGL(k_backsolve_w, dim3(n_dn), dim3(TPB), c.p_dn_lds, s, persist_plan(c), dn, c.d_pool.p, c.d_x.p, c.d_flags.p + c.flag_stride, c.d_bad.p, u);
         else
-            hipLaunchKernelGGL((k_backsolve_t<true>), dim3(c.p_dn_n), dim3(TPB), c.p_dn_lds, s, persist_plan(c), c.d_tab.p + c.p_dn_off, c.d_pool.p, c.d_x.p, 0, c.d_flags.p + c.flag_stride, 1, c.d_bad.p, u);
+            hipLaunchKernelGGL((k_backsolve_t<true>), dim3(n_dn), dim3(TPB), c.p_dn_lds, s, persist_plan(c), dn, c.d_pool.p, c.d_x.p, 0, c.d_flags.p + c.flag_stride, 1, c.d_bad.p, u);
         toc();
     }
     for (int l = l0 - 1; l >= 0; l--) {
         UpdArgs u = upd; if (l == 0) u.bad_out = io_host ? c.h_bad.p : nullptr;
         cur_level = l;
-        launch_backsolve(c, c.levels[l], s, tic, toc, nullptr, u);
+        if (l == 0 && c.x_leaf_n > 0) launch_backsolve(c, c.levels[0], s, tic, toc, nullptr, u, c.x_leaf_off, c.x_leaf_n);
+        else launch_backsolve(c, c.levels[l], s, tic, toc, nullptr, u);
     }
     if (ev) HIPCHECK(hipEventRecord(ev[3], s));
     HIPCHECK(hipGetLastError());
diff --git a/aprilsam_amd/csrc/symbolic.cpp b/aprilsam_amd/csrc/symbolic.cpp
--- a/aprilsam_amd/csrc/symbolic.cpp
+++ b/aprilsam_amd/csrc/symbolic.cpp
@@ -361,3 +361,106 @@
 }
 
 }
+
+namespace asam {
+
+XcdLists xcd_place(const std::vector<int> &up, const std::vector<int> &leaves, const int *parent, const int *nsb, int nF, int cap, int cap_leaf) {
+    constexpr int NX = 8;
+    const double HAND = 12.0, PERCOL = 0.19;
+    auto cost = [&](int t) { return HAND + PERCOL * 3.0 * (double)nsb[t]; };
+    XcdLists x;
+    const int n = (int)up.size();
+    std::vector<int> at((size_t)nF, -1);
+    for (int i = 0; i < n; i++) at[up[i]] = i;
+    auto up_parent = [&](int i) { const int p = parent[up[i]]; return p >= 0 ? at[p] : -1; };
+    std::vector<double> cp(n, 0.0), best(n, 0.0);
+    std::vector<int> heavy(n, -1);
+    for (int i = 0; i < n; i++) {
+        cp[i] = cost(up[i]) + best[i];
+        const int p = up_parent(i);
+        if (p >= 0 && (heavy[p] < 0 || cp[i] > best[p])) { best[p] = cp[i]; heavy[p] = i; }
+    }
+    std::vector<int> heads;
+    for (int i = 0; i < n; i++) { const int p = up_parent(i); if (p < 0 || heavy[p] != i) heads.push_back(i); }
+    std::stable_sort(heads.begin(), heads.end(), [&](int a, int b) { return cp[a] > cp[b]; });
+    std::vector<int> cls(n, 0), cnt(NX, 0);
+    std::vector<double> load(NX, 0.0);
+    const bool capped = n <= NX * cap;
+    auto room = [&](int c) { return !capped || cnt[c] < cap; };
+    auto emptiest = [&](const std::vector<int> &cn, const std::vector<double> &ld) {
+        int c = 0;
+        for (int k = 1; k < NX; k++) if (cn[k] < cn[c] || (cn[k] == cn[c] && ld[k] < ld[c])) c = k;
+        return c;
+    };
+    for (int h : heads) {
+        int c = emptiest(cnt, load);
+        for (int i = h; i >= 0; i = heavy[i]) {
+            while (!room(c)) c = (c + 1) % NX;
+            cls[i] = c; cnt[c]++; load[c] += cost(up[i]);
+        }
+    }
+    auto place = [&](bool down, std::vector<int> &list) {
+        std::vector<int> id(n, -1), dep(n, -1), cur(NX, 0);
+        int kmax = 0;
+        for (int j = 0; j < n; j++) {
+            const int i = down ? n - 1 - j : j, c = cls[i], p = up_parent(i);
+            const int need = (down ? (p >= 0 ? id[p] : -1) : dep[i]) + 1;
+            const int k = std::max(cur[c], need > c ? (need - c + NX - 1) / NX : 0);
+            id[i] = NX * k + c; cur[c] = k + 1; kmax = std::max(kmax, k + 1);
+            if (!down && p >= 0) dep[p] = std::max(dep[p], id[i]);
+        }
+        list.assign((size_t)NX * kmax, -1);
+        for (int i = 0; i < n; i++) list[id[i]] = up[i];
+    };
+    place(false, x.up);
+    place(true, x.dn);
+    std::vector<int> lv(leaves);
+    std::stable_sort(lv.begin(), lv.end(), [&](int a, int b) { return cost(a) > cost(b); });
+    std::vector<int> lcnt(NX, 0), lslot(lv.size());
+    std::vector<double> lload(NX, 0.0);
+    const bool lcapped = (long long)lv.size() <= (long long)NX * cap_leaf;
+    int kmax = 0;
+    for (size_t j = 0; j < lv.size(); j++) {
+        const int p = parent[lv[j]] >= 0 ? at[parent[lv[j]]] : -1;
+        int c = p >= 0 ? cls[p] : emptiest(lcnt, lload);
+        while (lcapped && lcnt[c] >= cap_leaf) c = (c + 1) % NX;
+        lslot[j] = NX * lcnt[c] + c; lcnt[c]++; lload[c] += cost(lv[j]); kmax = std::max(kmax, lcnt[c]);
+    }
+    x.leaf.assign((size_t)NX * kmax, -1);
+    for (size_t j = 0; j < lv.size(); j++) x.leaf[lslot[j]] = lv[j];
+    return x;
+}
+
+int xcd_check(const XcdLists &x, const std::vector<int> &up, const std::vector<int> &leaves, const int *parent, int nF, int cap, int cap_leaf) {
+    constexpr int NX = 8;
+    auto same_set = [&](const std::vector<int> &list, const std::vector<int> &old) {
+        if (list.size() % NX) return false;
+        std::vector<int> a, b(old);
+        for (int t : list) { if (t >= 0) a.push_back(t); else if (t != -1) return false; }
+        std::sort(a.begin(), a.end()); std::sort(b.begin(), b.end());
+        return a == b;
+    };
+    if (!same_set(x.up, up)) return -1;
+    if (!same_set(x.dn, up)) return -2;
+    if (!same_set(x.leaf, leaves)) return -3;
+    std::vector<int> iu((size_t)nF, -1), id((size_t)nF, -1);
+    for (size_t b = 0; b < x.up.size(); b++) if (x.up[b] >= 0) iu[x.up[b]] = (int)b;
+    for (size_t b = 0; b < x.dn.size(); b++) if (x.dn[b] >= 0) id[x.dn[b]] = (int)b;
+    for (int t : up) {
+        const int p = parent[t];
+        if (p >= 0 && iu[p] >= 0 && iu[t] >= iu[p]) return -4;
+        if (p >= 0 && id[p] >= 0 && id[t] <= id[p]) return -5;
+        if (iu[t] % NX != id[t] % NX) return -6;
+    }
+    auto fits = [&](const std::vector<int> &list, size_t n, int c) {
+        if (n > (size_t)NX * c) return true;
+        std::vector<int> cnt(NX, 0);
+        for (size_t b = 0; b < list.size(); b++) if (list[b] >= 0 && ++cnt[b % NX] > c) return false;
+        return true;
+    };
+    if (!fits(x.up, up.size(), cap) || !fits(x.dn, up.size(), cap)) return -7;
+    if (!fits(x.leaf, leaves.size(), cap_leaf)) return -8;
+    return 0;
+}
+
+}
diff --git a/include/aprilsam_amd.h b/include/aprilsam_amd.h
--- a/include/aprilsam_amd.h
+++ b/include/aprilsam_amd.h
@@ -246,6 +246,7 @@
 void aprilsam_amd_plan_destroy(aprilsam_amd_plan_t *plan);
 long long aprilsam_amd_plan_query(const aprilsam_amd_plan_t *plan, const char *what, long long **out);
 long long aprilsam_amd_shard_plan(const aprilsam_amd_plan_t *plan, int world, int what, long long *out, long long cap);
+int aprilsam_amd_xcd_place(int nF, const int *parent, const int *level, const int *nsb, int l0, int cap, int cap_leaf, int which, int *out, int out_cap);
 void aprilsam_amd_free(void *p);
 
 int aprilsam_amd_reference_order(int n_nodes, int n_factors, const int *fa, const int *fb, int *out_order, int *out_parent);
```

New measurement: 4788 GN iterations/s (median of 6 runs). 2.2% higher.
